# rsinghlab/GNN-Tumor-Seg

Measured on AMD Instinct MI355X. Metric: supervoxel-graphs/sec training, 7xSAGE-pool-256, 15k-node graphs, higher is better.
Workload: dtype f32

## Files before the change

gnn-tumor-seg_amd/csrc/gts_rows.h:

```cpp
#pragma once
#include <type_traits>

#include "gts_common.h"

namespace gts {

constexpr int kUnroll = 8;

__device__ __forceinline__ float mad(float w, float v, float acc) { return __builtin_fmaf(w, v, acc); }

typedef float v2f __attribute__((ext_vector_type(2)));
constexpr float kEluSplit = -0.35f, kLog2e = 1.44269504088896340736f;
constexpr float kEluC2 = 0.5f, kEluC3 = 1.0f / 6.0f, kEluC4 = 1.0f / 24.0f, kEluC5 = 1.0f / 120.0f, kEluC6 = 1.0f / 720.0f,
                kEluC7 = 1.0f / 5040.0f;
__device__ __forceinline__ float elu_expm1(float x) {
  float q = __builtin_fmaf(kEluC7, x, kEluC6);
  q = __builtin_fmaf(q, x, kEluC5);
  q = __builtin_fmaf(q, x, kEluC4);
  q = __builtin_fmaf(q, x, kEluC3);
  q = __builtin_fmaf(q, x, kEluC2);
  const float small = __builtin_fmaf(x * x, q, x);
  const float large = __builtin_amdgcn_exp2f(x * kLog2e) - 1.0f;
  return x < kEluSplit ? large : small;
}
__device__ __forceinline__ v2f elu_expm1_pair(v2f x) {
  v2f q = __builtin_elementwise_fma(v2f{kEluC7, kEluC7}, x, v2f{kEluC6, kEluC6});
  q = __builtin_elementwise_fma(q, x, v2f{kEluC5, kEluC5});
  q = __builtin_elementwise_fma(q, x, v2f{kEluC4, kEluC4});
  q = __builtin_elementwise_fma(q, x, v2f{kEluC3, kEluC3});
  q = __builtin_elementwise_fma(q, x, v2f{kEluC2, kEluC2});
  const v2f small = __builtin_elementwise_fma(x * x, q, x);
  const v2f arg = x * v2f{kLog2e, kLog2e};
  const v2f large = v2f{__builtin_amdgcn_exp2f(arg.x), __builtin_amdgcn_exp2f(arg.y)} - v2f{1.0f, 1.0f};
  return v2f{x.x < kEluSplit ? large.x : small.x, x.y < kEluSplit ? large.y : small.y};
}

template <int LPR>
__device__ __forceinline__ int owned_row(int s, int seq, int n_rows) {
  constexpr int kRowsPerWave = kWave / LPR;
  const int lane = threadIdx.x & (kWave - 1);
  const int wave = threadIdx.x / kWave;
  const int tile = xcd_contiguous_tile(blockIdx.x, gridDim.x);
  int v = ((tile * kWavesPerBlock + wave) * seq + s) * kRowsPerWave + lane / LPR;
  if constexpr (LPR == kWave) v = __builtin_amdgcn_readfirstlane(v);
  return v < n_rows ? v : -1;
}

template <int VEC, int LPR, typename Body>
__device__ __forceinline__ void for_columns(int n_feat, Body&& body) {
  const int gl = (threadIdx.x & (kWave - 1)) % LPR;
  for (int c0 = 0; c0 < n_feat; c0 += LPR * VEC) {
    const int c = c0 + gl * VEC;
    const bool active = c < n_feat;
    body(active ? c : 0, active);
  }
}

template <int N>
using IC = std::integral_constant<int, N>;

template <int LPR, typename Body>
__device__ __forceinline__ void for_chunks(int beg, int end, Body&& body) {
  if constexpr (LPR == kWave) {
    int k = beg;
    for (; k + kUnroll <= end; k += kUnroll) body(IC<kUnroll>{}, k);
    switch (end - k) {
      case 1: body(IC<1>{}, k); break;
      case 2: body(IC<2>{}, k); break;
      case 3: body(IC<3>{}, k); break;
      case 4: body(IC<4>{}, k); break;
      case 5: body(IC<5>{}, k); break;
      case 6: body(IC<6>{}, k); break;
      case 7: body(IC<7>{}, k); break;
      default: break;
    }
  } else {
    for (int k = beg; k < end; k += kUnroll) body(IC<kUnroll>{}, k);
  }
}

template <int LPR, int CNT>
struct Chunk {
  int reg;
  const int32_t* __restrict__ p;
  int k, last;
  __device__ __forceinline__ Chunk(const int32_t* __restrict__ arr, int k_, int end) : p(arr), k(k_), last(end - 1) {
    if constexpr (LPR == kWave) {
      const int lane = threadIdx.x & (kWave - 1);
      reg = lane < CNT ? arr[k_ + lane] : 0;
    } else {
      reg = 0;
    }
  }
  __device__ __forceinline__ int operator[](int j) const {
    if constexpr (LPR == kWave) {
      return __builtin_amdgcn_readlane(reg, j);
    } else {
      return p[min(k + j, last)];
    }
  }
  __device__ __forceinline__ bool valid(int j) const {
    if constexpr (LPR == kWave) return true;
    return k + j <= last;
  }
};

inline int g_spmm_seq = 0;
inline int g_project_nt = 1;
inline int g_spmm_nt = -1;
inline int g_cluster_nt = -1;
inline int g_gat_walk = 1;
inline int g_cluster_ring = 0;
inline int g_cluster_per_cu = 0;
inline int g_gat_cluster_waves = 0;
inline int g_cluster_dealing = 0;
inline int g_gat_cluster_dealing = 0;
inline int g_gat_cluster_group = 0;
inline int g_cluster_consumers = 0;

inline int pick_seq(int64_t n_rows, int rows_per_wave_step, int preferred) {
  if (g_spmm_seq > 0) return g_spmm_seq;
  if (preferred > 0) return preferred;
  const int64_t steps = (n_rows + rows_per_wave_step - 1) / rows_per_wave_step;
  int seq = 1;
  while (seq < 4 && steps / (seq * 2) >= 8192) seq *= 2;
  return seq;
}

struct Geometry {
  int vec, lpr, seq;
  dim3 grid;
};

inline Geometry make_geometry(int64_t n_rows, int64_t n_feat, int preferred_seq = 0) {
  Geometry g;
  g.vec = (n_feat % 4 == 0) ? 4 : 1;
  g.lpr = lanes_per_row(n_feat / g.vec);
  const int rows_per_step = kWave / g.lpr;
  g.seq = pick_seq(n_rows, rows_per_step, preferred_seq);
  const int64_t rows_per_block = static_cast<int64_t>(rows_per_step) * g.seq * kWavesPerBlock;
  g.grid = dim3(static_cast<unsigned>((n_rows + rows_per_block - 1) / rows_per_block));
  return g;
}

inline bool bad_shape(int64_t n_rows, int64_t n_feat) {
  return n_rows < 0 || n_feat <= 0 || n_rows >= (1LL << 31) || n_feat >= (1LL << 24);
}

}

#define GTS_DISPATCH_LPR(VEC_, LPR_VAL, ...)                \
  switch (LPR_VAL) {                                        \
    case 1: { constexpr int LPR = 1; __VA_ARGS__; } break;  \
    case 2: { constexpr int LPR = 2; __VA_ARGS__; } break;  \
    case 4: { constexpr int LPR = 4; __VA_ARGS__; } break;  \
    case 8: { constexpr int LPR = 8; __VA_ARGS__; } break;  \
    case 16: { constexpr int LPR = 16; __VA_ARGS__; } break; \
    case 32: { constexpr int LPR = 32; __VA_ARGS__; } break; \
    default: { constexpr int LPR = 64; __VA_ARGS__; } break; \
  }

#define GTS_DISPATCH_GEOM(G, ...)                                   \
  if ((G).vec == 4) {                                               \
    constexpr int VEC = 4;                                          \
    GTS_DISPATCH_LPR(4, (G).lpr, __VA_ARGS__)                       \
  } else {                                                          \
    constexpr int VEC = 1;                                          \
    GTS_DISPATCH_LPR(1, (G).lpr, __VA_ARGS__)                       \
  }
```

gnn-tumor-seg_amd/csrc/gts_spmm.hip:

```cpp
#include "gts_rows.h"

namespace gts {
namespace {

template <int ARGB>
struct ArgTraits;
template <>
struct ArgTraits<1> {
  using T = uint8_t;
  static constexpr int kNone = 0xFF;
};
template <>
struct ArgTraits<4> {
  using T = int32_t;
  static constexpr int kNone = -1;
};

template <int VEC, int ARGB>
__device__ __forceinline__ void store_slots(void* arg, size_t off, const int (&slot)[VEC]) {
  if constexpr (ARGB == 1) {
    uint8_t* p = static_cast<uint8_t*>(arg) + off;
    if constexpr (VEC == 4) {
      const uint32_t w = (slot[0] & 0xFF) | ((slot[1] & 0xFF) << 8) | ((slot[2] & 0xFF) << 16) |
                         (static_cast<uint32_t>(slot[3] & 0xFF) << 24);
      *reinterpret_cast<uint32_t*>(p) = w;
    } else {
      p[0] = static_cast<uint8_t>(slot[0]);
    }
  } else if constexpr (ARGB == 4) {
    int32_t* p = static_cast<int32_t*>(arg) + off;
    if constexpr (VEC == 4) {
      *reinterpret_cast<int4*>(p) = make_int4(slot[0], slot[1], slot[2], slot[3]);
    } else {
      p[0] = slot[0];
    }
  }
}

template <int VEC, int ARGB>
__device__ __forceinline__ void load_slots(const void* arg, size_t off, int (&slot)[VEC]) {
  if constexpr (ARGB == 1) {
    const uint8_t* p = static_cast<const uint8_t*>(arg) + off;
    if constexpr (VEC == 4) {
      const uint32_t w = *reinterpret_cast<const uint32_t*>(p);
      slot[0] = w & 0xFF;
      slot[1] = (w >> 8) & 0xFF;
      slot[2] = (w >> 16) & 0xFF;
      slot[3] = w >> 24;
    } else {
      slot[0] = p[0];
    }
  } else {
    const int32_t* p = static_cast<const int32_t*>(arg) + off;
    if constexpr (VEC == 4) {
      const int4 w = *reinterpret_cast<const int4*>(p);
      slot[0] = w.x, slot[1] = w.y, slot[2] = w.z, slot[3] = w.w;
    } else {
      slot[0] = p[0];
    }
  }
}

template <int VEC, int LPR, int ARGB>
__global__ __launch_bounds__(kBlock) void spmm_max_fwd_kernel(
    const int32_t* __restrict__ indptr, const int32_t* __restrict__ indices,
    const float* __restrict__ x, float* __restrict__ out, void* __restrict__ arg, int n_dst,
    int n_feat, int seq, int nt, int relu_input) {
  for (int s = 0; s < seq; ++s) {
    const int v = owned_row<LPR>(s, seq, n_dst);
    if (v < 0) continue;
    const int beg = indptr[v], end = indptr[v + 1];
    for_columns<VEC, LPR>(n_feat, [&](int c, bool active) {
      float best[VEC];
      int slot[VEC];
#pragma unroll
      for (int t = 0; t < VEC; ++t) best[t] = -INFINITY, slot[t] = -1;
      for_chunks<LPR>(beg, end, [&](auto cnt_c, int k) {
        constexpr int CNT = decltype(cnt_c)::value;
        const Chunk<LPR, CNT> src(indices, k, end);
        Vec<VEC> val[CNT];
#pragma unroll
        for (int j = 0; j < CNT; ++j)
          val[j] = Vec<VEC>::load(x + static_cast<size_t>(src[j]) * n_feat + c);
#pragma unroll
        for (int j = 0; j < CNT; ++j) {
          if (src.valid(j)) {
#pragma unroll
            for (int t = 0; t < VEC; ++t) {
              if (best[t] < val[j].v[t]) best[t] = val[j].v[t], slot[t] = k + j - beg;
            }
          }
        }
      });
      Vec<VEC> o;
#pragma unroll
      for (int t = 0; t < VEC; ++t) {
        const bool dead = isinf(best[t]);
        o.v[t] = dead ? 0.0f : best[t];
        slot[t] = (dead || (relu_input && !(best[t] > 0.0f))) ? -1 : slot[t];
      }
      const size_t off = static_cast<size_t>(v) * n_feat + c;
      if (active) {
        if (nt & 1) o.store_nt(out + off); else o.store(out + off);
        if constexpr (ARGB != 0) store_slots<VEC, ARGB>(arg, off, slot);
      }
    });
  }
}

template <int VEC, int LPR, int ARGB>
__global__ __launch_bounds__(kBlock) void spmm_max_bwd_kernel(
    const int32_t* __restrict__ t_indptr, const int32_t* __restrict__ t_indices,
    const int32_t* __restrict__ t_slot, const float* __restrict__ gout,
    const void* __restrict__ arg, const float* __restrict__ relu_src, float* __restrict__ gx,
    int n_src, int n_feat, int seq, int nt) {
  for (int s = 0; s < seq; ++s) {
    const int u = owned_row<LPR>(s, seq, n_src);
    if (u < 0) continue;
    const int beg = t_indptr[u], end = t_indptr[u + 1];
    for_columns<VEC, LPR>(n_feat, [&](int c, bool active) {
      float acc[VEC];
#pragma unroll
      for (int t = 0; t < VEC; ++t) acc[t] = 0.0f;
      for_chunks<LPR>(beg, end, [&](auto cnt_c, int k) {
        constexpr int CNT = decltype(cnt_c)::value;
        const Chunk<LPR, CNT> dst(t_indices, k, end);
        const Chunk<LPR, CNT> slt(t_slot, k, end);
        Vec<VEC> g[CNT];
        int win[CNT][VEC];
        int want[CNT];
#pragma unroll
        for (int j = 0; j < CNT; ++j) {
          const size_t off = static_cast<size_t>(dst[j]) * n_feat + c;
          want[j] = slt[j];
          g[j] = Vec<VEC>::load(gout + off);
          load_slots<VEC, ARGB>(arg, off, win[j]);
        }
#pragma unroll
        for (int j = 0; j < CNT; ++j) {
          if (dst.valid(j)) {
#pragma unroll
            for (int t = 0; t < VEC; ++t) acc[t] += (win[j][t] == want[j]) ? g[j].v[t] : 0.0f;
          }
        }
      });
      const size_t off = static_cast<size_t>(u) * n_feat + c;
      Vec<VEC> o;
      if (relu_src != nullptr) {
        const Vec<VEC> p = (nt & 2) ? Vec<VEC>::load_nt(relu_src + off) : Vec<VEC>::load(relu_src + off);
#pragma unroll
        for (int t = 0; t < VEC; ++t) o.v[t] = p.v[t] > 0.0f ? acc[t] : 0.0f;
      } else {
#pragma unroll
        for (int t = 0; t < VEC; ++t) o.v[t] = acc[t];
      }
      if (active) { if (nt & 1) o.store_nt(gx + off); else o.store(gx + off); }
    });
  }
}

template <int VEC, int LPR, bool DIV_IN>
__global__ __launch_bounds__(kBlock) void spmm_sum_kernel(
    const int32_t* __restrict__ indptr, const int32_t* __restrict__ indices,
    const float* __restrict__ x, float* __restrict__ out, const float* __restrict__ div_in,
    const float* __restrict__ div_out, const float* __restrict__ accum, int add_self, int n_out, int n_feat,
    int seq) {
  for (int s = 0; s < seq; ++s) {
    const int v = owned_row<LPR>(s, seq, n_out);
    if (v < 0) continue;
    const int beg = indptr[v], end = indptr[v + 1];
    for_columns<VEC, LPR>(n_feat, [&](int c, bool active) {
      float acc[VEC];
#pragma unroll
      for (int t = 0; t < VEC; ++t) acc[t] = 0.0f;
      for_chunks<LPR>(beg, end, [&](auto cnt_c, int k) {
        constexpr int CNT = decltype(cnt_c)::value;
        const Chunk<LPR, CNT> src(indices, k, end);
        Vec<VEC> val[CNT];
        float d[CNT];
#pragma unroll
        for (int j = 0; j < CNT; ++j) {
          const int u = src[j];
          d[j] = DIV_IN ? div_in[u] : 1.0f;
          val[j] = Vec<VEC>::load(x + static_cast<size_t>(u) * n_feat + c);
        }
#pragma unroll
        for (int j = 0; j < CNT; ++j) {
          if (src.valid(j)) {
#pragma unroll
            for (int t = 0; t < VEC; ++t) acc[t] += DIV_IN ? val[j].v[t] / d[j] : val[j].v[t];
          }
        }
      });
      const size_t off = static_cast<size_t>(v) * n_feat + c;
      if (add_self) {
        const Vec<VEC> self = Vec<VEC>::load(x + off);
        const float d = DIV_IN ? div_in[v] : 1.0f;
#pragma unroll
        for (int t = 0; t < VEC; ++t) acc[t] += DIV_IN ? self.v[t] / d : self.v[t];
      }
      Vec<VEC> o;
      const float dv = div_out != nullptr ? div_out[v] : 1.0f;
#pragma unroll
      for (int t = 0; t < VEC; ++t) o.v[t] = div_out != nullptr ? acc[t] / dv : acc[t];
      if (accum != nullptr) {
        const Vec<VEC> other = Vec<VEC>::load(accum + off);
#pragma unroll
        for (int t = 0; t < VEC; ++t) o.v[t] = other.v[t] + o.v[t];
      }
      if (active) o.store(out + off);
    });
  }
}

}
}

extern "C" int32_t gts_spmm_max_fwd_f32(const int32_t* indptr, const int32_t* indices,
                                        const float* x, float* out, void* arg,
                                        int32_t arg_bytes, int32_t relu_input, int64_t n_dst,
                                        int64_t n_feat, void* stream) {
  using namespace gts;
  if (!indptr || !x || !out || (arg_bytes != 0 && !arg)) return GTS_ERR_NULL;
  if (bad_shape(n_dst, n_feat)) return GTS_ERR_SHAPE;
  if (arg_bytes != 0 && arg_bytes != 1 && arg_bytes != 4) return GTS_ERR_ARGKIND;
  if (n_dst == 0) return GTS_OK;
  const Geometry g = make_geometry(n_dst, n_feat, 2);
  const int nt = g_spmm_nt < 0 ? 1 : g_spmm_nt;
  hipStream_t st = static_cast<hipStream_t>(stream);
  const int nd = static_cast<int>(n_dst), nf = static_cast<int>(n_feat);
  GTS_DISPATCH_GEOM(g, {
    if (arg_bytes == 0)
      spmm_max_fwd_kernel<VEC, LPR, 0><<<g.grid, kBlock, 0, st>>>(indptr, indices, x, out, arg, nd, nf, g.seq, nt, relu_input);
    else if (arg_bytes == 1)
      spmm_max_fwd_kernel<VEC, LPR, 1><<<g.grid, kBlock, 0, st>>>(indptr, indices, x, out, arg, nd, nf, g.seq, nt, relu_input);
    else
      spmm_max_fwd_kernel<VEC, LPR, 4><<<g.grid, kBlock, 0, st>>>(indptr, indices, x, out, arg, nd, nf, g.seq, nt, relu_input);
  })
  return launch_status();
}

extern "C" int32_t gts_spmm_max_bwd_f32(const int32_t* t_indptr, const int32_t* t_indices,
                                        const int32_t* t_slot, const float* gout,
                                        const void* arg, int32_t arg_bytes,
                                        const float* relu_src, float* gx, int64_t n_src,
                                        int64_t n_feat, void* stream) {
  using namespace gts;
  if (!t_indptr || !gout || !arg || !gx) return GTS_ERR_NULL;
  if (bad_shape(n_src, n_feat)) return GTS_ERR_SHAPE;
  if (arg_bytes != 1 && arg_bytes != 4) return GTS_ERR_ARGKIND;
  if (n_src == 0) return GTS_OK;
  const Geometry g = make_geometry(n_src, n_feat, 1);
  const int nt = g_spmm_nt < 0 ? 0 : g_spmm_nt;
  hipStream_t st = static_cast<hipStream_t>(stream);
  const int ns = static_cast<int>(n_src), nf = static_cast<int>(n_feat);
  GTS_DISPATCH_GEOM(g, {
    if (arg_bytes == 1)
      spmm_max_bwd_kernel<VEC, LPR, 1><<<g.grid, kBlock, 0, st>>>(t_indptr, t_indices, t_slot, gout, arg, relu_src, gx, ns, nf, g.seq, nt);
    else
      spmm_max_bwd_kernel<VEC, LPR, 4><<<g.grid, kBlock, 0, st>>>(t_indptr, t_indices, t_slot, gout, arg, relu_src, gx, ns, nf, g.seq, nt);
  })
  return launch_status();
}

extern "C" int32_t gts_spmm_sum_f32(const int32_t* indptr, const int32_t* indices,
                                    const float* x, float* out, const float* div_in,
                                    const float* div_out, const float* accum, int32_t add_self,
                                    int64_t n_out, int64_t n_feat, void* stream) {
  using namespace gts;
  if (!indptr || !x || !out) return GTS_ERR_NULL;
  if (bad_shape(n_out, n_feat)) return GTS_ERR_SHAPE;
  if (n_out == 0) return GTS_OK;
  const Geometry g = make_geometry(n_out, n_feat);
  hipStream_t st = static_cast<hipStream_t>(stream);
  const int no = static_cast<int>(n_out), nf = static_cast<int>(n_feat);
  GTS_DISPATCH_GEOM(g, {
    if (div_in != nullptr)
      spmm_sum_kernel<VEC, LPR, true><<<g.grid, kBlock, 0, st>>>(indptr, indices, x, out, div_in, div_out, accum, add_self, no, nf, g.seq);
    else
      spmm_sum_kernel<VEC, LPR, false><<<g.grid, kBlock, 0, st>>>(indptr, indices, x, out, div_in, div_out, accum, add_self, no, nf, g.seq);
  })
  return launch_status();
}
```

gnn-tumor-seg_amd/csrc/gts_spmm_cluster.hip:

```cpp
#include <algorithm>
#include <queue>
#include <vector>

#include "gts_cluster.h"

namespace gts {
namespace {

struct ClusterArgs {
  const int32_t* rec;
  RecLayout layout;
  int n_clusters, max_srcs;
  const float* table;
  const uint8_t* winners;
  float* out;
  uint8_t* arg;
  unsigned table_bytes, winners_bytes;
  int relu_input, nt;
  int ring, slot_bytes, image_off, win_off;
  int deal_off;
  unsigned* counters;
};

template <int ARGB, int WHATIF = 0>
__device__ __forceinline__ int reduce_max_rows(const ClusterArgs& a, const int32_t* l_rec, const unsigned char* image,
                                               int part, int first, int step) {
  const int lane = threadIdx.x & (kWave - 1), half = lane >> 5, hl = lane & 31;
  const int n_rows = l_rec[0];
  const uint32_t* info = reinterpret_cast<const uint32_t*>(l_rec + a.layout.eoff);
  const uint2* loc = reinterpret_cast<const uint2*>(l_rec + a.layout.loc);
  const unsigned char* mine = image + hl * 16;
  int trips = 0;
  for (int j0 = 2 * first; j0 < n_rows; j0 += 2 * step, ++trips) {
    const int j = j0 + half;
    const bool have = j < n_rows;
    const uint32_t ri = have ? info[j] : 0u;
    const int c0 = ri & 0xFFFF, deg = ri >> 16;
    const int deg_w = max(__builtin_amdgcn_readlane(deg, 0), __builtin_amdgcn_readlane(deg, 32));
    float best[4];
    int slot[4];
#pragma unroll
    for (int t = 0; t < 4; ++t) best[t] = -INFINITY, slot[t] = -1;
    for (int c = 0; 8 * c < deg_w && WHATIF != 4; ++c) {
      const bool mine_too = 8 * c < deg;
      const uint2 w = loc[mine_too ? c0 + c : c0];
      for_count(min(8, deg_w - 8 * c), [&](auto cnt_c) {
        constexpr int CNT = decltype(cnt_c)::value;
        constexpr int FIRST = CNT > 6 ? 6 : CNT;
        float4 val[FIRST];
#pragma unroll
        for (int q = 0; q < FIRST; ++q) val[q] = *reinterpret_cast<const float4*>(mine + chunk_byte(w, q) * kHalfBytes);
#pragma unroll
        for (int q = 0; q < FIRST; ++q) {
          const float v4[4] = {val[q].x, val[q].y, val[q].z, val[q].w};
#pragma unroll
          for (int t = 0; t < 4; ++t) {
            const bool up = mine_too && best[t] < v4[t];
            best[t] = up ? v4[t] : best[t];
            slot[t] = up ? 8 * c + q : slot[t];
          }
        }
        if constexpr (CNT > FIRST) {
          float4 rest[CNT - FIRST];
#pragma unroll
          for (int q = FIRST; q < CNT; ++q) rest[q - FIRST] = *reinterpret_cast<const float4*>(mine + chunk_byte(w, q) * kHalfBytes);
#pragma unroll
          for (int q = FIRST; q < CNT; ++q) {
            const float v4[4] = {rest[q - FIRST].x, rest[q - FIRST].y, rest[q - FIRST].z, rest[q - FIRST].w};
#pragma unroll
            for (int t = 0; t < 4; ++t) {
              const bool up = mine_too && best[t] < v4[t];
              best[t] = up ? v4[t] : best[t];
              slot[t] = up ? 8 * c + q : slot[t];
            }
          }
        }
      });
    }
    Vec<4> o;
#pragma unroll
    for (int t = 0; t < 4; ++t) {
      const bool dead = isinf(best[t]);
      o.v[t] = dead ? 0.0f : best[t];
      slot[t] = (dead || (a.relu_input && !(best[t] > 0.0f))) ? -1 : slot[t];
    }
    if (WHATIF == 3) {
      if (o.v[0] == 123.456f) a.out[0] = static_cast<float>(slot[0] + slot[1] + slot[2] + slot[3]) + o.v[1] + o.v[2] + o.v[3];
    } else if (have) {
      const size_t off = static_cast<size_t>(l_rec[a.layout.rows + j]) * kF + part * (kF / 2) + hl * 4;
      if (a.nt & 1) o.store_nt(a.out + off); else o.store(a.out + off);
      if constexpr (ARGB == 1) {
        const uint32_t w = (slot[0] & 0xFF) | ((slot[1] & 0xFF) << 8) | ((slot[2] & 0xFF) << 16) |
                           (static_cast<uint32_t>(slot[3] & 0xFF) << 24);
        *reinterpret_cast<uint32_t*>(a.arg + off) = w;
      }
    }
  }
  return trips * (ARGB == 1 ? 2 : 1);
}

__device__ __forceinline__ int reduce_winner_rows(const ClusterArgs& a, const int32_t* l_rec, const unsigned char* image,
                                                  const unsigned char* winners, int part, int first, int step) {
  const int lane = threadIdx.x & (kWave - 1), half = lane >> 5, hl = lane & 31;
  const int n_rows = l_rec[0];
  const uint32_t* info = reinterpret_cast<const uint32_t*>(l_rec + a.layout.eoff);
  const uint2* loc = reinterpret_cast<const uint2*>(l_rec + a.layout.loc);
  const uint2* tag = reinterpret_cast<const uint2*>(l_rec + a.layout.tag);
  const unsigned char* my_g = image + hl * 16;
  const unsigned char* my_w = winners + hl * 4;
  int trips = 0;
  for (int j0 = 2 * first; j0 < n_rows; j0 += 2 * step, ++trips) {
    const int j = j0 + half;
    const bool have = j < n_rows;
    const uint32_t ri = have ? info[j] : 0u;
    const int c0 = ri & 0xFFFF, deg = ri >> 16;
    const int deg_a = __builtin_amdgcn_readlane(deg, 0), deg_b = __builtin_amdgcn_readlane(deg, 32);
    const int deg_w = max(deg_a, deg_b);
    float acc[4] = {0.f, 0.f, 0.f, 0.f};
    if (deg_a == deg_b && deg_w <= 8) {
      if (deg_w > 0) {
        const uint2 w = loc[c0], tg = tag[c0];
        for_count(deg_w, [&](auto cnt_c) {
          constexpr int CNT = decltype(cnt_c)::value;
          constexpr int FIRST = CNT > 6 ? 6 : CNT;
          auto group = [&](auto q0_c, auto n_c) {
            constexpr int Q0 = decltype(q0_c)::value, N = decltype(n_c)::value;
            float4 g[N];
            uint32_t win[N];
#pragma unroll
            for (int q = 0; q < N; ++q) {
              const unsigned s = chunk_byte(w, Q0 + q);
              g[q] = *reinterpret_cast<const float4*>(my_g + s * kHalfBytes);
              win[q] = *reinterpret_cast<const uint32_t*>(my_w + s * kArgHalfBytes);
            }
#pragma unroll
            for (int q = 0; q < N; ++q) {
              const unsigned want = chunk_byte(tg, Q0 + q);
              acc[0] += (win[q] & 0xFF) == want ? g[q].x : 0.0f;
              acc[1] += ((win[q] >> 8) & 0xFF) == want ? g[q].y : 0.0f;
              acc[2] += ((win[q] >> 16) & 0xFF) == want ? g[q].z : 0.0f;
              acc[3] += (win[q] >> 24) == want ? g[q].w : 0.0f;
            }
          };
          group(IC<0>{}, IC<FIRST>{});
          if constexpr (CNT > FIRST) group(IC<FIRST>{}, IC<CNT - FIRST>{});
        });
      }
    } else {
      for (int c = 0; 8 * c < deg_w; ++c) {
        const int at = 8 * c < deg ? c0 + c : c0;
        const uint2 w = loc[at], tg = tag[at];
        for_count(min(8, deg_w - 8 * c), [&](auto cnt_c) {
          constexpr int CNT = decltype(cnt_c)::value;
          constexpr int FIRST = CNT > 6 ? 6 : CNT;
          auto group = [&](auto q0_c, auto n_c) {
            constexpr int Q0 = decltype(q0_c)::value, N = decltype(n_c)::value;
            float4 g[N];
            uint32_t win[N];
#pragma unroll
            for (int q = 0; q < N; ++q) {
              const unsigned s = chunk_byte(w, Q0 + q);
              g[q] = *reinterpret_cast<const float4*>(my_g + s * kHalfBytes);
              win[q] = *reinterpret_cast<const uint32_t*>(my_w + s * kArgHalfBytes);
            }
#pragma unroll
            for (int q = 0; q < N; ++q) {
              const unsigned want = chunk_byte(tg, Q0 + q);
              const bool live = 8 * c + Q0 + q < deg;
              const float g4[4] = {g[q].x, g[q].y, g[q].z, g[q].w};
#pragma unroll
              for (int t = 0; t < 4; ++t) acc[t] += (live && ((win[q] >> (8 * t)) & 0xFF) == want) ? g4[t] : 0.0f;
            }
          };
          group(IC<0>{}, IC<FIRST>{});
          if constexpr (CNT > FIRST) group(IC<FIRST>{}, IC<CNT - FIRST>{});
        });
      }
    }
    if (have) {
      const size_t off = static_cast<size_t>(l_rec[a.layout.rows + j]) * kF + part * (kF / 2) + hl * 4;
      const Vec<4> o{{acc[0], acc[1], acc[2], acc[3]}};
      if (a.nt & 1) o.store_nt(a.out + off); else o.store(a.out + off);
    }
  }
  return trips;
}

template <typename Dma, typename SrcOf>
__device__ __forceinline__ void gather_winner_halves(const Dma& dma, int part, unsigned char* image,
                                                     int n_srcs, int first, int step, SrcOf&& src_of) {
  const int l8 = threadIdx.x & 7;
  for (int i = first; i < n_srcs; i += step) {
    const unsigned voff = static_cast<unsigned>(src_of(i)) * static_cast<unsigned>(kF) +
                          static_cast<unsigned>(part) * kArgHalfBytes + l8 * 16u;
    dma(image + i * kArgHalfBytes, voff);
  }
}

template <bool BWD, int ARGB, int WHATIF = 0, int DEPTH = 1, bool DEAL = false>
__global__ __launch_bounds__(1024, BWD ? 6 : 8) void spmm_cluster_stream_kernel(const ClusterArgs a) {
  extern __shared__ __attribute__((aligned(16))) unsigned char lds[];
  const int lane = threadIdx.x & (kWave - 1);
  const int wave = __builtin_amdgcn_readfirstlane(threadIdx.x / kWave);
  const int n_waves = blockDim.x / kWave;
  const int xcd = blockIdx.x & 7, j = blockIdx.x >> 3, per_xcd = gridDim.x >> 3;
  const long long n_units = 2LL * a.n_clusters;
  const int lo = static_cast<int>(n_units * xcd / 8), hi = static_cast<int>(n_units * (xcd + 1) / 8);
  constexpr bool dynamic = DEAL;
  const int n_static = lo + j < hi ? (hi - lo - j + per_xcd - 1) / per_xcd : 0;
  if (!dynamic && n_static == 0) return;
  const int clo = static_cast<int>(static_cast<long long>(a.n_clusters) * xcd / 8);
  const int span = static_cast<int>(static_cast<long long>(a.n_clusters) * (xcd + 1) / 8) - clo;
  const int words = a.layout.words;
  const int pieces = (words + 255) / 256;
  const int rec_bytes = 1024 * pieces, image_bytes = a.slot_bytes - a.image_off;
  constexpr int depth = DEPTH, n_images = DEPTH + 1, n_recs = DEPTH + 2;
  unsigned char* images = lds + n_recs * rec_bytes;
  const RawDma rr(a.rec, static_cast<unsigned>(a.n_clusters) * words * 4u);
  const RawDma rt(a.table, a.table_bytes);
  const RawDma rw(a.winners, BWD ? a.winners_bytes : 0);
  constexpr int PIPE = DEPTH + 2;
  int u_unit[dynamic ? PIPE : 1];
#pragma unroll
  for (int q = 0; q < (dynamic ? PIPE : 1); ++q) u_unit[q] = -1;
  int32_t* l_deal = reinterpret_cast<int32_t*>(lds + a.deal_off);
  auto next_unit = [&](int deal_slot) {
    if constexpr (dynamic) {
#pragma unroll
      for (int q = PIPE - 1; q > 0; --q) u_unit[q] = u_unit[q - 1];
      const unsigned idx = static_cast<unsigned>(__builtin_amdgcn_readfirstlane(l_deal[deal_slot]));
      const unsigned part = idx >= static_cast<unsigned>(span) ? 1u : 0u;
      u_unit[0] = idx < 2u * static_cast<unsigned>(span) ? static_cast<int>(((clo + idx - part * span) << 1) | part) : -1;
    }
  };
  auto unit_at = [&](int k, int newest) {
    if constexpr (dynamic) {
      return u_unit[k];
    } else {
      const int t = newest - k;
      return t < n_static ? lo + j + t * per_xcd : -1;
    }
  };
  auto take = [&](int count) {
    unsigned base = 0;
    if (lane == 0) base = __hip_atomic_fetch_add(a.counters + 32 * xcd, static_cast<unsigned>(count), __ATOMIC_RELAXED, __HIP_MEMORY_SCOPE_AGENT);
    return base;
  };
  auto publish = [&](unsigned taken, int count, int slot0) {
    if (lane == 0) {
      for (int q = 0; q < count; ++q) l_deal[slot0 + q] = static_cast<int>(taken + q);
    }
  };
  auto fetch_record = [&](int t, int unit) {
    if (wave < pieces) {
      const unsigned cluster = static_cast<unsigned>(unit) >> 1;
      const int word = 256 * wave + 4 * lane;
      const unsigned voff = word < words ? (cluster * static_cast<unsigned>(words) + word) * 4u : 0xFFFFFFF0u;
      rr(lds + (t % n_recs) * rec_bytes + 1024 * wave, voff);
    }
  };
  auto issue_gathers = [&](int t, int unit) {
    const int32_t* l_rec = reinterpret_cast<const int32_t*>(lds + (t % n_recs) * rec_bytes);
    unsigned char* image = images + (t % n_images) * image_bytes;
    const int n_srcs = l_rec[1];
    const int part = unit & 1;
    const int half = lane >> 5;
    const int last = pad4(a.max_srcs) - 1;
    const int32_t ids = l_rec[a.layout.srcs + min(2 * (wave + n_waves * (lane >> 1)) + (lane & 1), last)];
    int k = 0;
    gather_halves(rt, part, image, n_srcs, 2 * wave, 2 * n_waves, [&](int) {
      const int s0 = __builtin_amdgcn_readlane(ids, 2 * k), s1 = __builtin_amdgcn_readlane(ids, 2 * k + 1);
      ++k;
      return half ? s1 : s0;
    });
    if constexpr (BWD) {
      const int32_t ids8 = l_rec[a.layout.srcs + min(8 * (wave + n_waves * (lane >> 3)) + (lane & 7), last)];
      int k8 = 0;
      gather_winner_halves(rw, part, image + ((a.max_srcs + 1) & ~1) * kHalfBytes, n_srcs, 8 * wave, 8 * n_waves, [&](int) {
        const int32_t id = __builtin_amdgcn_ds_bpermute(4 * (8 * k8 + (lane >> 3)), ids8);
        ++k8;
        return id;
      });
      return k + k8;
    }
    return k;
  };

  if constexpr (dynamic) {
    if (wave == n_waves - 1) {
      const unsigned first = take(PIPE);
      publish(first, PIPE - 1, 0);
      publish(first + (PIPE - 1), 1, 6);
    }
    barrier_all();
  }
  unsigned taken = 0;
#pragma unroll
  for (int t = 0; t <= depth; ++t) {
    next_unit(t);
    if (unit_at(0, t) >= 0) fetch_record(t, unit_at(0, t));
  }
  barrier_all();
  int pending_gathers = 0, stores = 0;
#pragma unroll
  for (int t = 0; t < depth; ++t) pending_gathers = (WHATIF != 1 && unit_at(depth - t, depth) >= 0) ? issue_gathers(t, unit_at(depth - t, depth)) : 0;
  if (depth == 1) pending_gathers = 0;
  unsigned long long phase[4] = {0, 0, 0, 0}, stamp = 0;
  auto lap = [&](int which) {
    if constexpr (WHATIF == 9) {
      const unsigned long long now = __builtin_amdgcn_s_memtime();
      phase[which] += now - stamp;
      stamp = now;
    }
  };
  if constexpr (WHATIF == 9) stamp = __builtin_amdgcn_s_memtime();
  int it = 0;
  for (; dynamic || it < n_static; ++it) {
    wait_vm_all_but(pending_gathers + stores);
    if constexpr (dynamic) {
      if (it > 0 && wave == n_waves - 1) publish(taken, 1, 6 + (it & 1));
    }
    lap(0);
    barrier_lds();
    lap(1);
    next_unit(6 + (it & 1));
    const int newest = it + depth + 1;
    const int unit_now = unit_at(PIPE - 1, newest);
    if constexpr (dynamic) {
      if (unit_now < 0) break;
    }
    if constexpr (dynamic) {
      if (wave == n_waves - 1) taken = take(1);
    }
    if constexpr (DEPTH == 1) {
      if (unit_at(1, newest) >= 0 && WHATIF != 1) issue_gathers(it + 1, unit_at(1, newest));
      if (unit_at(0, newest) >= 0) fetch_record(it + 2, unit_at(0, newest));
    } else {
      if (unit_at(0, newest) >= 0) fetch_record(it + depth + 1, unit_at(0, newest));
      pending_gathers = (unit_at(1, newest) >= 0 && WHATIF != 1) ? issue_gathers(it + depth, unit_at(1, newest)) : 0;
    }
    lap(2);
    const int32_t* l_rec = reinterpret_cast<const int32_t*>(lds + (it % n_recs) * rec_bytes);
    const unsigned char* image = images + (it % n_images) * image_bytes;
    const int part = unit_now & 1;
    if constexpr (WHATIF == 2)
      stores = 0;
    else if constexpr (WHATIF >= 3 && WHATIF <= 4 && !BWD)
      stores = WHATIF == 3 ? (reduce_max_rows<ARGB, WHATIF>(a, l_rec, image, part, wave, n_waves), 0)
                           : reduce_max_rows<ARGB, WHATIF>(a, l_rec, image, part, wave, n_waves);
    else if constexpr (BWD)
      stores = reduce_winner_rows(a, l_rec, image, image + ((a.max_srcs + 1) & ~1) * kHalfBytes, part, wave, n_waves);
    else
      stores = reduce_max_rows<ARGB>(a, l_rec, image, part, wave, n_waves);
    lap(3);
  }
  if constexpr (WHATIF == 9) {
    if (threadIdx.x == 0) {
      unsigned long long* dbg = reinterpret_cast<unsigned long long*>(a.arg) + 8 * static_cast<size_t>(blockIdx.x);
      for (int q = 0; q < 4; ++q) dbg[q] = phase[q];
      dbg[4] = static_cast<unsigned long long>(it);
    }
  }
  if (dynamic && threadIdx.x == 0) {
    unsigned* done = a.counters + 32 * xcd + 16;
    if (__hip_atomic_fetch_add(done, 1u, __ATOMIC_RELAXED, __HIP_MEMORY_SCOPE_AGENT) == static_cast<unsigned>(per_xcd) - 1u) {
      __hip_atomic_store(a.counters + 32 * xcd, 0u, __ATOMIC_RELAXED, __HIP_MEMORY_SCOPE_AGENT);
      __hip_atomic_store(done, 0u, __ATOMIC_RELAXED, __HIP_MEMORY_SCOPE_AGENT);
    }
  }
}

struct LdsPlan {
  int slot_bytes, image_off, win_off;
};
inline LdsPlan lds_plan(int max_rows, int max_srcs, int loc_words, bool bwd) {
  const RecLayout l = rec_layout(max_rows, max_srcs, loc_words, bwd);
  LdsPlan p;
  p.image_off = (l.words * 4 + 15) & ~15;
  const int image = ((max_srcs + 1) & ~1) * kHalfBytes;
  p.win_off = p.image_off + image;
  p.slot_bytes = p.win_off + (bwd ? ((max_srcs + 7) & ~7) * kArgHalfBytes : 0);
  return p;
}

struct ClusterGeometry {
  int64_t wg_lds, grid;
  int depth, waves;
  bool deals;
};
inline ClusterGeometry cluster_geometry(int64_t n_clusters, int words, int slot_bytes, int image_off, bool bwd, bool whatif) {
  ClusterGeometry g;
  const int64_t units = 2LL * n_clusters;
  const int64_t rec_slot = 1024LL * ((words + 255) / 256), image = slot_bytes - image_off;
  g.depth = (g_cluster_ring == 2 && !whatif && 4 * rec_slot + 3 * image + 64 <= kMaxLds) ? 2 : 1;
  g.wg_lds = (g.depth + 2) * rec_slot + (g.depth + 1) * image + 64;
  g.waves = g_cluster_consumers > 0 ? std::min(16, g_cluster_consumers) : (bwd ? 12 : 16);
  const int auto_per_cu = (bwd && units <= 24LL * device_cus()) ? 3 : 2;
  const int per_cu = static_cast<int>(std::max<int64_t>(1, std::min<int64_t>(g_cluster_per_cu > 0 ? g_cluster_per_cu : auto_per_cu, kMaxLds / std::max<int64_t>(1, g.wg_lds))));
  g.grid = static_cast<int64_t>(device_cus()) * per_cu;
  g.grid = std::max<int64_t>(8, std::min(g.grid, (units + 7) / 8 * 8)) / 8 * 8;
  g.deals = g_cluster_dealing == 1 || (g_cluster_dealing == 0 && units >= 16 * g.grid);
  return g;
}

template <bool BWD, int ARGB, int WHATIF = 0>
inline int launch_cluster(ClusterArgs a, int max_rows, int loc_words, hipStream_t st) {
  const LdsPlan p = lds_plan(max_rows, a.max_srcs, loc_words, BWD);
  a.image_off = p.image_off, a.win_off = p.win_off, a.slot_bytes = p.slot_bytes;
  if (p.slot_bytes > kMaxLds) return GTS_ERR_SHAPE;
  const int64_t units = 2LL * a.n_clusters;
  {
    const ClusterGeometry geo = cluster_geometry(a.n_clusters, a.layout.words, p.slot_bytes, p.image_off, BWD, WHATIF != 0);
    const int depth = geo.depth, waves = geo.waves;
    const int64_t wg_lds = geo.wg_lds, grid = geo.grid;
    a.deal_off = static_cast<int>(wg_lds) - 64;
    if (wg_lds > kMaxLds || a.layout.words > 512) return GTS_ERR_SHAPE;
    a.ring = depth;
    if (a.max_srcs > 64 * waves) return GTS_ERR_SHAPE;
    if (!geo.deals) a.counters = nullptr;
    static const bool once = (allow_big_lds(spmm_cluster_stream_kernel<BWD, ARGB, WHATIF, 1, false>),
                              allow_big_lds(spmm_cluster_stream_kernel<BWD, ARGB, WHATIF, 1, true>),
                              allow_big_lds(spmm_cluster_stream_kernel<BWD, ARGB, WHATIF == 0 ? 0 : WHATIF, WHATIF == 0 ? 2 : 1, false>),
                              allow_big_lds(spmm_cluster_stream_kernel<BWD, ARGB, WHATIF == 0 ? 0 : WHATIF, WHATIF == 0 ? 2 : 1, true>), true);
    (void)once;
    const dim3 g3(static_cast<unsigned>(grid));
    if constexpr (WHATIF == 0) {
      if (depth == 2) {
        if (a.counters != nullptr) spmm_cluster_stream_kernel<BWD, ARGB, 0, 2, true><<<g3, waves * kWave, wg_lds, st>>>(a);
        else spmm_cluster_stream_kernel<BWD, ARGB, 0, 2, false><<<g3, waves * kWave, wg_lds, st>>>(a);
        return launch_status();
      }
    }
    if (a.counters != nullptr) spmm_cluster_stream_kernel<BWD, ARGB, WHATIF, 1, true><<<g3, waves * kWave, wg_lds, st>>>(a);
    else spmm_cluster_stream_kernel<BWD, ARGB, WHATIF, 1, false><<<g3, waves * kWave, wg_lds, st>>>(a);
    return launch_status();
  }
}

}
}

extern "C" int64_t gts_cluster_record_words(int32_t max_rows, int32_t max_srcs, int32_t loc_words, int32_t with_tag) {
  if (max_rows < 1 || max_srcs < 1 || loc_words < 0 || loc_words % 4 != 0) return -1;
  return gts::rec_layout(max_rows, max_srcs, loc_words, with_tag != 0).words;
}

extern "C" int32_t gts_cluster_schedule(const int32_t* indptr, const int32_t* indices, const int32_t* t_indptr,
                                        const int32_t* t_indices, const int32_t* edge_tag, int64_t n_rows,
                                        int32_t max_rows, int32_t max_srcs, int32_t max_edges, int32_t* rec,
                                        int64_t rec_capacity, int64_t* n_clusters, int64_t* n_staged,
                                        int32_t* max_cluster_edges) {
  using namespace gts;
  if (!indptr || !t_indptr || !n_clusters || !n_staged || !max_cluster_edges) return GTS_ERR_NULL;
  if (n_rows < 0 || n_rows >= (1LL << 31)) return GTS_ERR_SHAPE;
  if (max_rows < 1 || max_srcs < 1 || max_srcs > 256 || max_edges < 1 || max_edges > 65535) return GTS_ERR_ARGKIND;
  const int n = static_cast<int>(n_rows);
  if (n > 0 && (!indices || !t_indices) && indptr[n] > 0) return GTS_ERR_NULL;
  if (n > 0) {
    if (indptr[0] != 0 || t_indptr[0] != 0) return GTS_ERR_SHAPE;
    for (int v = 0; v < n; ++v)
      if (indptr[v + 1] < indptr[v] || t_indptr[v + 1] < t_indptr[v]) return GTS_ERR_SHAPE;
    if (indptr[n] != t_indptr[n]) return GTS_ERR_SHAPE;
    const int e_all = indptr[n];
    for (int k = 0; k < e_all; ++k)
      if (indices[k] < 0 || indices[k] >= n || t_indices[k] < 0 || t_indices[k] >= n) return GTS_ERR_SHAPE;
  }
  for (int v = 0; v < n; ++v) {
    const int deg = indptr[v + 1] - indptr[v];
    if (deg > max_srcs || ((deg + 7) & ~7) > max_edges || deg > 65535) return GTS_ERR_SHAPE;
  }
  if (edge_tag != nullptr) {
    const int e = n > 0 ? indptr[n] : 0;
    for (int k = 0; k < e; ++k)
      if (edge_tag[k] < 0 || edge_tag[k] > 255) return GTS_ERR_SHAPE;
  }
  const int loc_words = pad4((max_edges + 3) / 4);
  const RecLayout L = rec_layout(max_rows, max_srcs, loc_words, edge_tag != nullptr);
  if (L.words > 64 * kRecRegs) return GTS_ERR_ARGKIND;
  std::vector<uint8_t> assigned(n, 0);
  std::vector<int> gain(n, 0), stamp(n, -1);
  std::vector<int> local(n, -1), lstamp(n, -1);
  using Cand = std::pair<int, int>;
  std::priority_queue<Cand> heap;
  std::priority_queue<int, std::vector<int>, std::greater<int>> seeds;
  std::vector<int> rows, srcs, touched;
  int next_unassigned = 0, most_edges = 0;
  int64_t n_cl = 0, staged = 0;
  while (true) {
    int seed = -1;
    while (!seeds.empty()) {
      const int s = seeds.top();
      seeds.pop();
      if (!assigned[s]) { seed = s; break; }
    }
    if (seed < 0) {
      while (next_unassigned < n && assigned[next_unassigned]) ++next_unassigned;
      if (next_unassigned == n) break;
      seed = next_unassigned;
    }
    const int cl = static_cast<int>(n_cl);
    rows.clear(), srcs.clear(), touched.clear();
    int n_e = 0;
    while (!heap.empty()) heap.pop();
    heap.push({0, -seed});
    stamp[seed] = cl, gain[seed] = 0;
    bool full = false, misfit = false;
    while (!full) {
      if (heap.empty()) {
        if (misfit) break;
        while (next_unassigned < n && assigned[next_unassigned]) ++next_unassigned;
        if (next_unassigned == n) break;
        const int s = next_unassigned;
        if (stamp[s] != cl) stamp[s] = cl, gain[s] = 0;
        heap.push({gain[s], -s});
      }
      const Cand top = heap.top();
      heap.pop();
      const int v = -top.second;
      if (assigned[v] || stamp[v] != cl || gain[v] != top.first) continue;
      const int beg = indptr[v], end = indptr[v + 1];
      int fresh = 0;
      for (int k = beg; k < end; ++k) {
        const int u = indices[k];
        if (lstamp[u] != cl) lstamp[u] = cl, local[u] = -1;
        if (local[u] == -1) local[u] = -2, ++fresh;
      }
      const int padded = (end - beg + 7) & ~7;
      const bool fits = static_cast<int>(rows.size()) < max_rows &&
                        static_cast<int>(srcs.size()) + fresh <= max_srcs && n_e + padded <= max_edges;
      if (!fits) {
        for (int k = beg; k < end; ++k)
          if (local[indices[k]] == -2) local[indices[k]] = -1;
        if (rows.empty()) return GTS_ERR_SHAPE;
        misfit = true;
        continue;
      }
      assigned[v] = 1;
      rows.push_back(v);
      n_e += padded;
      for (int k = beg; k < end; ++k) {
        const int u = indices[k];
        if (local[u] != -2) continue;
        local[u] = static_cast<int>(srcs.size());
        srcs.push_back(u);
        for (int q = t_indptr[u]; q < t_indptr[u + 1]; ++q) {
          const int w = t_indices[q];
          if (assigned[w]) continue;
          if (stamp[w] != cl) stamp[w] = cl, gain[w] = 0, touched.push_back(w);
          ++gain[w];
          heap.push({gain[w], -w});
        }
      }
      if (static_cast<int>(rows.size()) >= max_rows) full = true;
    }
    for (int w : touched)
      if (!assigned[w]) seeds.push(w);
    most_edges = std::max(most_edges, n_e);
    staged += static_cast<int64_t>(srcs.size());
    if (rec != nullptr && n_cl < rec_capacity) {
      std::sort(rows.begin(), rows.end());
      int32_t* r = rec + n_cl * L.words;
      std::fill(r, r + L.words, 0);
      r[0] = static_cast<int32_t>(rows.size()), r[1] = static_cast<int32_t>(srcs.size()), r[2] = n_e;
      uint8_t* loc = reinterpret_cast<uint8_t*>(r + L.loc);
      uint8_t* tag = reinterpret_cast<uint8_t*>(r + L.tag);
      int e_at = 0;
      for (size_t i = 0; i < rows.size(); ++i) {
        const int v = rows[i], deg = indptr[v + 1] - indptr[v];
        r[L.rows + i] = v;
        r[L.eoff + i] = static_cast<int32_t>(static_cast<uint32_t>(e_at / 8) | (static_cast<uint32_t>(deg) << 16));
        for (int k = indptr[v]; k < indptr[v + 1]; ++k, ++e_at) {
          loc[e_at] = static_cast<uint8_t>(local[indices[k]]);
          if (edge_tag != nullptr) tag[e_at] = static_cast<uint8_t>(edge_tag[k]);
        }
        for (; e_at % 8 != 0; ++e_at) {
          loc[e_at] = loc[e_at - 1];
          if (edge_tag != nullptr) tag[e_at] = tag[e_at - 1];
        }
      }
      for (int i = 0; i < pad4(max_srcs); ++i)
        r[L.srcs + i] = srcs.empty() ? 0 : srcs[std::min<size_t>(i, srcs.size() - 1)];
    }
    ++n_cl;
  }
  *n_clusters = n_cl;
  *n_staged = staged;
  *max_cluster_edges = most_edges;
  return GTS_OK;
}

extern "C" int64_t gts_cluster_lds_bytes(int32_t max_rows, int32_t max_srcs, int32_t loc_words, int32_t kind) {
  if (max_rows < 1 || max_srcs < 1 || loc_words < 0 || loc_words % 4 != 0 || (kind != 0 && kind != 1)) return -1;
  return gts::lds_plan(max_rows, max_srcs, loc_words, kind == 1).slot_bytes;
}

namespace {
inline bool bad_cluster_shape(int64_t n_clusters, int32_t max_rows, int32_t max_srcs, int32_t loc_words, bool tag,
                              int64_t n_rows, int64_t n_feat) {
  if (n_feat != gts::kF || n_rows < 0 || n_rows * gts::kF * 4 >= (1LL << 32) || n_clusters < 0 || n_clusters >= (1 << 30))
    return true;
  if (max_rows < 1 || max_srcs < 1 || max_srcs > 256 || loc_words < 0 || loc_words % 4 != 0 || loc_words > 16384) return true;
  return gts::rec_layout(max_rows, max_srcs, loc_words, tag).words > 64 * gts::kRecRegs;
}
}

extern "C" int32_t gts_cluster_uses_counters(int64_t n_clusters, int32_t max_rows, int32_t max_srcs, int32_t loc_words, int32_t backward) {
  using namespace gts;
  if (n_clusters <= 0 || max_rows < 1 || max_srcs < 1 || loc_words < 0) return 0;
  const LdsPlan p = lds_plan(max_rows, max_srcs, loc_words, backward != 0);
  return cluster_geometry(n_clusters, rec_layout(max_rows, max_srcs, loc_words, backward != 0).words, p.slot_bytes, p.image_off, backward != 0, false).deals ? 1 : 0;
}

extern "C" int32_t gts_spmm_max_fwd_cluster_f32(const int32_t* rec, int64_t n_clusters, int32_t max_rows, int32_t max_srcs,
                                                int32_t loc_words, const float* x, float* out, void* arg,
                                                int32_t arg_bytes, int32_t relu_input, int64_t n_rows, int64_t n_feat,
                                                uint32_t* counters, void* stream) {
  using namespace gts;
  if (!rec || !x || !out || (arg_bytes != 0 && !arg)) return GTS_ERR_NULL;
  if (bad_cluster_shape(n_clusters, max_rows, max_srcs, loc_words, false, n_rows, n_feat)) return GTS_ERR_SHAPE;
  if (arg_bytes != 0 && arg_bytes != 1) return GTS_ERR_ARGKIND;
  if (n_clusters == 0) return GTS_OK;
  ClusterArgs a{};
  a.rec = rec, a.layout = rec_layout(max_rows, max_srcs, loc_words, false);
  a.n_clusters = static_cast<int>(n_clusters), a.max_srcs = max_srcs;
  a.table = x, a.out = out, a.arg = static_cast<uint8_t*>(arg), a.counters = counters;
  a.table_bytes = static_cast<unsigned>(n_rows * kF * 4);
  a.relu_input = relu_input, a.nt = g_cluster_nt < 0 ? 1 : g_cluster_nt;
  hipStream_t st = static_cast<hipStream_t>(stream);
  return arg_bytes == 0 ? launch_cluster<false, 0>(a, max_rows, loc_words, st) : launch_cluster<false, 1>(a, max_rows, loc_words, st);
}

extern "C" int32_t gts_spmm_max_bwd_cluster_f32(const int32_t* rec, int64_t n_clusters, int32_t max_rows, int32_t max_srcs,
                                                int32_t loc_words, const float* gout, const void* arg, int32_t arg_bytes,
                                                float* gx, int64_t n_rows, int64_t n_feat, uint32_t* counters, void* stream) {
  using namespace gts;
  if (!rec || !gout || !arg || !gx) return GTS_ERR_NULL;
  if (bad_cluster_shape(n_clusters, max_rows, max_srcs, loc_words, true, n_rows, n_feat)) return GTS_ERR_SHAPE;
  if (arg_bytes != 1) return GTS_ERR_ARGKIND;
  if (n_clusters == 0) return GTS_OK;
  ClusterArgs a{};
  a.rec = rec, a.layout = rec_layout(max_rows, max_srcs, loc_words, true);
  a.n_clusters = static_cast<int>(n_clusters), a.max_srcs = max_srcs;
  a.table = gout, a.winners = static_cast<const uint8_t*>(arg), a.out = gx, a.counters = counters;
  a.table_bytes = static_cast<unsigned>(n_rows * kF * 4), a.winners_bytes = static_cast<unsigned>(n_rows * kF);
  a.nt = g_cluster_nt < 0 ? 1 : g_cluster_nt;
  return launch_cluster<true, 1>(a, max_rows, loc_words, static_cast<hipStream_t>(stream));
}
```

gnn-tumor-seg_amd/csrc/gts_stack.hip:

```cpp
#include <algorithm>
#include <vector>

#include "gts_common.h"

namespace {

constexpr int kMaxLayers = 64;
constexpr int kMaxWgradProblems = 32;
constexpr int kFlagChain = 1, kFlagReluBits = 2, kFlagTransposedIgrad = 4;

inline int64_t align256(int64_t bytes) { return (bytes + 255) & ~255LL; }

inline bool bad_stack(int64_t n_rows, const int64_t* widths, int32_t n_layers) {
  if (!widths || n_layers < 1 || n_layers > kMaxLayers || n_rows < 0 || n_rows >= (1LL << 31)) return true;
  for (int i = 0; i <= n_layers; ++i)
    if (widths[i] <= 0 || widths[i] % 4 != 0 || widths[i] >= (1 << 20)) return true;
  return false;
}

struct FwdPlan {
  int64_t m[kMaxLayers], arg[kMaxLayers], out[kMaxLayers], bits[kMaxLayers];
  int64_t p[2];
  int64_t wp[kMaxLayers][3];
  int64_t counters;
  int64_t total;
};

inline bool packs(int64_t out_cols) { return out_cols > 128; }

inline FwdPlan plan_forward(int64_t n, const int64_t* w, int n_layers, bool training, int arg_bytes, int flags) {
  FwdPlan p{};
  int64_t at = 0, widest = 0;
  auto take = [&](int64_t bytes) { const int64_t o = at; at += align256(bytes); return o; };
  for (int i = 0; i < n_layers; ++i) {
    const bool last = i == n_layers - 1;
    widest = std::max(widest, w[i]);
    p.m[i] = take(4 * n * w[i]);
    p.arg[i] = training ? take(static_cast<int64_t>(arg_bytes) * n * w[i]) : -1;
    p.out[i] = take(4 * n * w[i + 1]);
    const bool bits = (flags & kFlagReluBits) && training && !last && gts_relu_bits_pay(n, w[i + 1]) == 1;
    p.bits[i] = bits ? take(gts_relu_bits_bytes(n, w[i + 1])) : -1;
  }
  p.p[0] = take(4 * n * widest);
  p.p[1] = take(4 * n * widest);
  for (int i = 0; i < n_layers; ++i) {
    p.wp[i][0] = packs(w[i]) ? take(4 * gts_packed_weight_floats(w[i], w[i])) : -1;
    p.wp[i][1] = packs(w[i + 1]) ? take(4 * gts_packed_weight_floats(w[i + 1], w[i])) : -1;
    p.wp[i][2] = packs(w[i + 1]) ? take(4 * gts_packed_weight_floats(w[i + 1], w[i])) : -1;
  }
  p.counters = take(4 * GTS_CLUSTER_COUNTER_WORDS);
  p.total = at;
  return p;
}

inline bool chainable(int64_t n, int64_t k0, int64_t k1, int64_t n2) {
  return n % 4 == 0 && k0 % 4 == 0 && k1 % 4 == 0 && n <= 256 && n2 <= 256;
}

struct Schedule {
  const int32_t* rec;
  int64_t clusters;
  int32_t rows, srcs, loc_words;
};

inline bool turns(int64_t rows, int64_t cols) { return cols >= 128 && rows % 4 == 0 && cols % 4 == 0; }

struct BwdPlan {
  int64_t wt[kMaxLayers][3];
  int64_t wtp[kMaxLayers][3];
  int64_t g[kMaxLayers], gp[kMaxLayers];
  int64_t gm[2];
  int64_t workspace, workspace_bytes;
  int64_t counters;
  int64_t total;
};

struct WgradGroup {
  int64_t n, k;
  std::vector<const float*> g, a;
  std::vector<float*> gw, gb;
};

inline BwdPlan plan_backward(int64_t n, const int64_t* w, int n_layers, int flags) {
  BwdPlan p{};
  int64_t at = 0, widest = 0;
  auto take = [&](int64_t bytes) { const int64_t o = at; at += align256(bytes); return o; };
  const bool t = (flags & kFlagTransposedIgrad) != 0;
  for (int i = 0; i < n_layers; ++i) {
    const int64_t fin = w[i], fout = w[i + 1];
    widest = std::max(widest, fin);
    p.wt[i][0] = t && turns(fin, fin) ? take(4 * fin * fin) : -1;
    p.wt[i][1] = t && turns(fout, fin) ? take(4 * fout * fin) : -1;
    p.wt[i][2] = t && turns(fout, fin) ? take(4 * fout * fin) : -1;
    p.wtp[i][0] = p.wt[i][0] >= 0 ? take(4 * gts_packed_weight_floats(fin, fin)) : -1;
    p.wtp[i][1] = p.wt[i][1] >= 0 ? take(4 * gts_packed_weight_floats(fin, fout)) : -1;
    p.wtp[i][2] = p.wt[i][2] >= 0 ? take(4 * gts_packed_weight_floats(fin, fout)) : -1;
    p.g[i] = i > 0 ? take(4 * n * fin) : -1;
    p.gp[i] = take(4 * n * fin);
  }
  p.gm[0] = take(4 * n * widest);
  p.gm[1] = take(4 * n * widest);
  struct Key { int64_t n, k; int count; };
  std::vector<Key> groups;
  auto add = [&](int64_t nn, int64_t kk) {
    for (auto& gk : groups)
      if (gk.n == nn && gk.k == kk) { ++gk.count; return; }
    groups.push_back({nn, kk, 1});
  };
  for (int i = n_layers - 1; i >= 0; --i) add(w[i], w[i]), add(w[i + 1], w[i]), add(w[i + 1], w[i]);
  int64_t ws = 0;
  if (n > 0)
    for (const auto& gk : groups)
      for (int first = 0; first < gk.count; first += kMaxWgradProblems)
        ws = std::max(ws, gts_linear_bwd_weight_workspace(n, gk.n, gk.k, std::min(kMaxWgradProblems, gk.count - first)));
  p.workspace_bytes = ws;
  p.workspace = take(ws);
  p.counters = take(4 * GTS_CLUSTER_COUNTER_WORDS);
  p.total = at;
  return p;
}

#define GTS_TRY(call)                    \
  do {                                   \
    const int32_t code_ = (call);        \
    if (code_ != GTS_OK) return code_;   \
  } while (0)

}

extern "C" int64_t gts_sage_pool_stack_fwd_arena(int64_t n_rows, const int64_t* widths, int32_t n_layers, int32_t training,
                                                 int32_t arg_bytes, int32_t flags, int64_t* offsets) {
  if (bad_stack(n_rows, widths, n_layers) || (training && arg_bytes != 1 && arg_bytes != 4)) return -1;
  const FwdPlan p = plan_forward(n_rows, widths, n_layers, training != 0, arg_bytes, flags);
  if (offsets != nullptr) {
    for (int i = 0; i < n_layers; ++i)
      offsets[4 * i] = p.m[i], offsets[4 * i + 1] = p.arg[i], offsets[4 * i + 2] = p.out[i], offsets[4 * i + 3] = p.bits[i];
    offsets[4 * n_layers] = p.p[0], offsets[4 * n_layers + 1] = p.p[1];
  }
  return p.total;
}

extern "C" int32_t gts_sage_pool_stack_fwd_f32(const int32_t* indptr, const int32_t* indices, const int32_t* sched_rec,
                                               int64_t sched_clusters, int32_t sched_rows, int32_t sched_srcs,
                                               int32_t sched_loc_words, const float* x, const float* const* params,
                                               int64_t n_rows, const int64_t* widths, int32_t n_layers, int32_t training,
                                               int32_t arg_bytes, int32_t flags, void* arena, int64_t arena_bytes,
                                               void* stream) {
  if (!indptr || !x || !params || !arena) return GTS_ERR_NULL;
  if (bad_stack(n_rows, widths, n_layers)) return GTS_ERR_SHAPE;
  if (training && arg_bytes != 1 && arg_bytes != 4) return GTS_ERR_ARGKIND;
  for (int i = 0; i < 5 * n_layers; ++i)
    if (!params[i]) return GTS_ERR_NULL;
  const bool train = training != 0;
  const FwdPlan plan = plan_forward(n_rows, widths, n_layers, train, arg_bytes, flags);
  if (arena_bytes < plan.total) return GTS_ERR_SHAPE;
  if (n_rows == 0) return GTS_OK;
  char* base = static_cast<char*>(arena);
  auto f32 = [&](int64_t off) { return reinterpret_cast<float*>(base + off); };
  uint32_t* counters = nullptr;
  if (sched_rec != nullptr && gts_cluster_uses_counters(sched_clusters, sched_rows, sched_srcs, sched_loc_words, 0) != 0) {
    counters = reinterpret_cast<uint32_t*>(base + plan.counters);
    if (hipMemsetAsync(counters, 0, 4 * GTS_CLUSTER_COUNTER_WORDS, static_cast<hipStream_t>(stream)) != hipSuccess) return GTS_ERR_SHAPE;
  }
  {
    struct Batch { int64_t rows, cols; std::vector<const float*> src; std::vector<float*> dst; };
    std::vector<Batch> batches;
    for (int i = 0; i < n_layers; ++i) {
      const int64_t fin = widths[i], fout = widths[i + 1];
      const int64_t shape[3][2] = {{fin, fin}, {fout, fin}, {fout, fin}};
      const int which[3] = {0, 2, 3};
      for (int q = 0; q < 3; ++q) {
        if (plan.wp[i][q] < 0) continue;
        Batch* b = nullptr;
        for (auto& c : batches)
          if (c.rows == shape[q][0] && c.cols == shape[q][1]) b = &c;
        if (b == nullptr) batches.push_back({shape[q][0], shape[q][1], {}, {}}), b = &batches.back();
        b->src.push_back(params[5 * i + which[q]]);
        b->dst.push_back(f32(plan.wp[i][q]));
      }
    }
    for (const auto& b : batches)
      GTS_TRY(gts_pack_weights_f32(b.src.data(), b.dst.data(), nullptr, static_cast<int32_t>(b.src.size()), b.rows, b.cols, 0,
                                   stream));
  }
  auto wp = [&](int i, int q) -> const float* { return plan.wp[i][q] >= 0 ? f32(plan.wp[i][q]) : nullptr; };
  const float* h = x;
  float* p = nullptr;
  int cur = 0;
  for (int i = 0; i < n_layers; ++i) {
    const float* w_pool = params[5 * i];
    const float* b_pool = params[5 * i + 1];
    const float* w_self = params[5 * i + 2];
    const float* w_neigh = params[5 * i + 3];
    const float* bias = params[5 * i + 4];
    const int64_t fin = widths[i], fout = widths[i + 1];
    const bool last = i == n_layers - 1;
    if (p == nullptr) {
      p = f32(plan.p[cur]);
      const float* packed[2] = {wp(i, 0), nullptr};
      GTS_TRY(gts_linear_fwd_f32(h, w_pool, nullptr, nullptr, b_pool, p, n_rows, fin, fin, 0, 1, nullptr, packed, stream));
    }
    float* m = f32(plan.m[i]);
    void* arg = train ? static_cast<void*>(base + plan.arg[i]) : nullptr;
    const int ab = train ? arg_bytes : 0;
    if (sched_rec != nullptr && fin == 256 && ab != 4 && n_rows * 1024 < (1LL << 32)) {
      GTS_TRY(gts_spmm_max_fwd_cluster_f32(sched_rec, sched_clusters, sched_rows, sched_srcs, sched_loc_words, p, m, arg, ab,
                                           1, n_rows, fin, counters, stream));
    } else {
      GTS_TRY(gts_spmm_max_fwd_f32(indptr, indices, p, m, arg, ab, 1, n_rows, fin, stream));
    }
    uint64_t* bits = plan.bits[i] >= 0 ? reinterpret_cast<uint64_t*>(base + plan.bits[i]) : nullptr;
    float* out = f32(plan.out[i]);
    if ((flags & kFlagChain) && !last && chainable(fout, fin, fin, fout)) {
      float* p_next = f32(plan.p[cur ^ 1]);
      const float* packed[3] = {wp(i, 1), wp(i, 2), wp(i + 1, 0)};
      GTS_TRY(gts_linear_fwd_chain_f32(h, w_self, m, w_neigh, bias, out, params[5 * (i + 1)], params[5 * (i + 1) + 1], p_next,
                                       n_rows, fout, fin, fin, 1, fout, 1, bits, packed, stream));
      p = p_next, cur ^= 1;
    } else {
      const float* packed[2] = {wp(i, 1), wp(i, 2)};
      GTS_TRY(gts_linear_fwd_f32(h, w_self, m, w_neigh, bias, out, n_rows, fout, fin, fin, last ? 0 : 1, bits, packed, stream));
      p = nullptr;
    }
    h = out;
  }
  return GTS_OK;
}

extern "C" int64_t gts_sage_pool_stack_bwd_scratch(int64_t n_rows, const int64_t* widths, int32_t n_layers, int32_t flags) {
  if (bad_stack(n_rows, widths, n_layers)) return -1;
  return plan_backward(n_rows, widths, n_layers, flags).total;
}

extern "C" int32_t gts_sage_pool_stack_bwd_f32(const int32_t* t_indptr, const int32_t* t_indices, const int32_t* t_slot,
                                               const int32_t* sched_rec, int64_t sched_clusters, int32_t sched_rows,
                                               int32_t sched_srcs, int32_t sched_loc_words, const float* gout, const float* x,
                                               const float* const* params, int64_t n_rows, const int64_t* widths,
                                               int32_t n_layers, int32_t arg_bytes, int32_t flags, const void* fwd_arena,
                                               float* const* grads, float* gx, void* scratch, int64_t scratch_bytes,
                                               void* stream) {
  if (!t_indptr || !gout || !x || !params || !fwd_arena || !grads || !scratch) return GTS_ERR_NULL;
  if (bad_stack(n_rows, widths, n_layers)) return GTS_ERR_SHAPE;
  if (arg_bytes != 1 && arg_bytes != 4) return GTS_ERR_ARGKIND;
  for (int i = 0; i < 5 * n_layers; ++i)
    if (!params[i] || !grads[i]) return GTS_ERR_NULL;
  hipStream_t st = static_cast<hipStream_t>(stream);
  if (n_rows == 0) {
    for (int i = 0; i < n_layers; ++i) {
      const int64_t fin = widths[i], fout = widths[i + 1];
      const int64_t sizes[5] = {fin * fin, fin, fout * fin, fout * fin, fout};
      for (int q = 0; q < 5; ++q)
        if (hipMemsetAsync(grads[5 * i + q], 0, 4 * sizes[q], st) != hipSuccess) return gts::launch_status();
    }
    return GTS_OK;
  }
  const FwdPlan fwd = plan_forward(n_rows, widths, n_layers, true, arg_bytes, flags);
  const BwdPlan plan = plan_backward(n_rows, widths, n_layers, flags);
  if (scratch_bytes < plan.total) return GTS_ERR_SHAPE;
  const char* acts = static_cast<const char*>(fwd_arena);
  char* base = static_cast<char*>(scratch);
  auto f32 = [&](int64_t off) { return reinterpret_cast<float*>(base + off); };
  uint32_t* counters = nullptr;
  if (sched_rec != nullptr && gts_cluster_uses_counters(sched_clusters, sched_rows, sched_srcs, sched_loc_words, 1) != 0) {
    counters = reinterpret_cast<uint32_t*>(base + plan.counters);
    if (hipMemsetAsync(counters, 0, 4 * GTS_CLUSTER_COUNTER_WORDS, static_cast<hipStream_t>(stream)) != hipSuccess) return GTS_ERR_SHAPE;
  }
  auto act = [&](int64_t off) { return reinterpret_cast<const float*>(acts + off); };
  auto input_of = [&](int i) { return i == 0 ? x : act(fwd.out[i - 1]); };

  {
    struct Batch { int64_t rows, cols; std::vector<const float*> src; std::vector<float*> dst, packed; };
    std::vector<Batch> batches;
    for (int i = 0; i < n_layers; ++i) {
      const int64_t fin = widths[i], fout = widths[i + 1];
      const int64_t shape[3][2] = {{fin, fin}, {fout, fin}, {fout, fin}};
      const int which[3] = {0, 2, 3};
      for (int q = 0; q < 3; ++q) {
        if (plan.wt[i][q] < 0) continue;
        Batch* b = nullptr;
        for (auto& c : batches)
          if (c.rows == shape[q][0] && c.cols == shape[q][1]) b = &c;
        if (b == nullptr) batches.push_back({shape[q][0], shape[q][1], {}, {}, {}}), b = &batches.back();
        b->src.push_back(params[5 * i + which[q]]);
        b->dst.push_back(f32(plan.wt[i][q]));
        b->packed.push_back(f32(plan.wtp[i][q]));
      }
    }
    for (const auto& b : batches)
      GTS_TRY(gts_pack_weights_f32(b.src.data(), b.packed.data(), b.dst.data(), static_cast<int32_t>(b.src.size()), b.rows,
                                   b.cols, 1, stream));
  }
  auto wt = [&](int i, int q) -> const float* { return plan.wt[i][q] >= 0 ? f32(plan.wt[i][q]) : nullptr; };
  auto wtp = [&](int i, int q) -> const float* { return plan.wtp[i][q] >= 0 ? f32(plan.wtp[i][q]) : nullptr; };

  auto igrad = [&](const float* g0, const float* w0, const float* w0t, int64_t n0, const float* g1, const float* w1,
                   const float* w1t, int64_t n1, const float* relu_mask, const uint64_t* relu_bits, float* gin,
                   int64_t k, const float* w0tp, const float* w1tp) -> int32_t {
    if (w0t != nullptr && (g1 == nullptr || w1t != nullptr)) {
      const float* packed[2] = {w0tp, g1 ? w1tp : nullptr};
      return gts_linear_bwd_input_t_f32(g0, w0t, g1, g1 ? w1t : nullptr, relu_mask, relu_mask ? relu_bits : nullptr, gin,
                                        n_rows, k, n0, g1 ? n1 : 0, packed, stream);
    }
    return gts_linear_bwd_input_f32(g0, w0, g1, g1 ? w1 : nullptr, relu_mask, gin, n_rows, k, n0, g1 ? n1 : 0, stream);
  };

  std::vector<WgradGroup> groups;
  auto defer = [&](const float* g, int64_t n, const float* a, int64_t k, float* gw, float* gb) {
    WgradGroup* grp = nullptr;
    for (auto& c : groups)
      if (c.n == n && c.k == k) grp = &c;
    if (grp == nullptr) groups.push_back({n, k, {}, {}, {}, {}}), grp = &groups.back();
    grp->g.push_back(g), grp->a.push_back(a), grp->gw.push_back(gw), grp->gb.push_back(gb);
  };

  const float* g = gout;
  const float* gm = nullptr;
  int cur = 0;
  for (int i = n_layers - 1; i >= 0; --i) {
    const float* w_pool = params[5 * i];
    const float* w_self = params[5 * i + 2];
    const float* w_neigh = params[5 * i + 3];
    const int64_t fin = widths[i], fout = widths[i + 1];
    const float* h = input_of(i);
    const float* m = act(fwd.m[i]);
    const void* arg = acts + fwd.arg[i];
    if (gm == nullptr) {
      float* buf = f32(plan.gm[cur]);
      GTS_TRY(igrad(g, w_neigh, wt(i, 2), fout, nullptr, nullptr, nullptr, 0, nullptr, nullptr, buf, fin, wtp(i, 2), nullptr));
      gm = buf;
    }
    float* gp = f32(plan.gp[i]);
    if (sched_rec != nullptr && fin == 256 && arg_bytes == 1 && n_rows * 1024 < (1LL << 32)) {
      GTS_TRY(gts_spmm_max_bwd_cluster_f32(sched_rec, sched_clusters, sched_rows, sched_srcs, sched_loc_words, gm, arg, 1, gp,
                                           n_rows, fin, counters, stream));
    } else {
      GTS_TRY(gts_spmm_max_bwd_f32(t_indptr, t_indices, t_slot, gm, arg, arg_bytes, nullptr, gp, n_rows, fin, stream));
    }
    gm = nullptr;
    defer(gp, fin, h, fin, grads[5 * i], grads[5 * i + 1]);
    defer(g, fout, h, fin, grads[5 * i + 2], grads[5 * i + 4]);
    defer(g, fout, m, fin, grads[5 * i + 3], nullptr);
    if (i > 0) {
      const int64_t below_in = widths[i - 1];
      const uint64_t* hbits = fwd.bits[i - 1] >= 0 ? reinterpret_cast<const uint64_t*>(acts + fwd.bits[i - 1]) : nullptr;
      float* g_next = f32(plan.g[i]);
      const float* below_t = wt(i - 1, 2);
      if ((flags & kFlagChain) && wt(i, 1) && wt(i, 0) && below_t && chainable(fin, fout, fin, below_in)) {
        float* gm_next = f32(plan.gm[cur ^ 1]);
        const float* packed[3] = {wtp(i, 1), wtp(i, 0), wtp(i - 1, 2)};
        GTS_TRY(gts_linear_bwd_input_chain_t_f32(g, wt(i, 1), gp, wt(i, 0), h, hbits, g_next, below_t, gm_next, n_rows, fin,
                                                 fout, fin, below_in, packed, stream));
        gm = gm_next, cur ^= 1;
      } else {
        GTS_TRY(igrad(g, w_self, wt(i, 1), fout, gp, w_pool, wt(i, 0), fin, h, hbits, g_next, fin, wtp(i, 1), wtp(i, 0)));
      }
      g = g_next;
    } else if (gx != nullptr) {
      GTS_TRY(igrad(g, w_self, wt(i, 1), fout, gp, w_pool, wt(i, 0), fin, nullptr, nullptr, gx, fin, wtp(i, 1), wtp(i, 0)));
    }
  }
  for (const auto& grp : groups) {
    const int count = static_cast<int>(grp.g.size());
    for (int first = 0; first < count; first += kMaxWgradProblems) {
      const int q = std::min(kMaxWgradProblems, count - first);
      GTS_TRY(gts_linear_bwd_weight_f32(grp.g.data() + first, grp.a.data() + first, grp.gw.data() + first,
                                        grp.gb.data() + first, q, f32(plan.workspace), plan.workspace_bytes, n_rows, grp.n,
                                        grp.k, stream));
    }
  }
  return GTS_OK;
}
```

gnn-tumor-seg_amd/gts/nn.py:

```python
import os

import torch
import torch.nn as nn
import torch.nn.functional as F

from . import dense, ops


class GraphError(RuntimeError):
    """Counterpart of dgl.DGLError for the checks the layers make."""


def _is_relu(fn):
    return fn in (F.relu, torch.relu, torch.nn.functional.relu)


class _SagePoolLayer(torch.autograd.Function):

    @staticmethod
    def forward(ctx, g, h, w_pool, b_pool, w_self, w_neigh, bias, relu_out, need_bwd):
        h = h.contiguous()
        p = dense.linear_fwd(h, w_pool, bias=b_pool, relu=True)
        m, arg = ops.spmm_max_fwd(g, p, want_arg=need_bwd, relu_input=True)
        out = dense.linear_fwd(h, w_self, m, w_neigh, bias=bias, relu=relu_out)
        if need_bwd:
            ctx.g, ctx.relu_out = g, relu_out
            ctx.save_for_backward(h, m, arg, out if relu_out else None, w_pool, w_self, w_neigh)
        return out

    @staticmethod
    def backward(ctx, gout):
        h, m, arg, out, w_pool, w_self, w_neigh = ctx.saved_tensors
        if not ctx.relu_out:
            g = gout.contiguous()
        elif out.shape[1] % 4 == 0 and out.shape[0] > 0:
            g, _ = ops.gat_act_bwd(gout.contiguous(), out, 2, want_bias_grad=False)
        else:
            g = dense.relu_bwd(gout, out)
        need = ctx.needs_input_grad
        gm = dense.linear_bwd_input(g, w_neigh)
        gp = ops.spmm_max_bwd(ctx.g, gm, arg)
        g_ws, g_wn, g_wp, g_bias, g_bp = _pool_layer_weight_grads(g, gp, h, m, w_pool, w_self)
        gh = dense.linear_bwd_input(g, w_self, gp, w_pool) if need[1] else None
        return None, gh, g_wp, g_bp, g_ws, g_wn, g_bias, None, None


class _SageSumLayer(torch.autograd.Function):

    @staticmethod
    def forward(ctx, g, h, w_self, w_neigh, bias, mode, relu_out, need_bwd):
        h = h.contiguous()
        d = g.dev()
        fin, fout = w_neigh.shape[1], w_neigh.shape[0]
        lin_first = fin > fout
        div = d.deg_clamped if mode == "mean" else d.deg_plus1
        src = dense.linear_fwd(h, w_neigh) if lin_first else h
        neigh = ops.spmm_sum_raw(g, src, div_out=div, add_self=(mode == "gcn"))
        last_w = _identity(fout, h.device) if lin_first else w_neigh
        if w_self is not None:
            out = dense.linear_fwd(h, w_self, neigh, last_w, bias=bias, relu=relu_out)
        else:
            out = dense.linear_fwd(neigh, last_w, bias=bias, relu=relu_out)
        if need_bwd:
            ctx.g, ctx.mode, ctx.relu_out, ctx.lin_first = g, mode, relu_out, lin_first
            ctx.has_bias = bias is not None
            ctx.save_for_backward(h, neigh if not lin_first else None, out if relu_out else None, w_self, w_neigh)
        return out

    @staticmethod
    def backward(ctx, gout):
        h, neigh, out, w_self, w_neigh = ctx.saved_tensors
        g, mode = ctx.g, ctx.mode
        d = g.dev()
        div = d.deg_clamped if mode == "mean" else d.deg_plus1
        need = ctx.needs_input_grad
        g_pre, g_bias = ops.gat_act_bwd(gout.contiguous(), out, 2 if ctx.relu_out else 0, want_bias_grad=ctx.has_bias)

        def reduce_bwd(t, accum=None):
            return ops.spmm_sum_raw(g, t, transposed=True, div_in=div, add_self=(mode == "gcn"), accum=accum)

        g_ws = None
        if ctx.lin_first:
            gt = reduce_bwd(g_pre)
            if w_self is not None:
                (g_ws, _), (g_wn, _) = dense.linear_bwd_weight_multi([(g_pre, h, False), (gt, h, False)])
                gh = dense.linear_bwd_input(g_pre, w_self, gt, w_neigh) if need[1] else None
            else:
                g_wn, _ = dense.linear_bwd_weight(gt, h)
                gh = dense.linear_bwd_input(gt, w_neigh) if need[1] else None
        else:
            if w_self is not None:
                (g_ws, _), (g_wn, _) = dense.linear_bwd_weight_multi([(g_pre, h, False), (g_pre, neigh, False)])
            else:
                g_wn, _ = dense.linear_bwd_weight(g_pre, neigh)
            gh = None
            if need[1]:
                gneigh = dense.linear_bwd_input(g_pre, w_neigh)
                gself = dense.linear_bwd_input(g_pre, w_self) if w_self is not None else None
                gh = reduce_bwd(gneigh, accum=gself)
        return None, gh, g_ws, g_wn, g_bias, None, None, None


_identities = {}


def _identity(n, device):
    key = (n, device)
    if key not in _identities:
        _identities[key] = torch.eye(n, dtype=torch.float32, device=device)
    return _identities[key]


OVERLAP_WEIGHT_GRADS = os.environ.get("GTS_OVERLAP_WGRAD", "0") != "0"
TRANSPOSED_IGRAD = os.environ.get("GTS_TRANSPOSED_IGRAD", "1") != "0"
_side_streams = {}


def _side_stream(device):
    s = _side_streams.get(device)
    if s is None:
        try:
            priority = torch.cuda.Stream.priority_range()[0]
        except Exception:
            priority = 0
        s = torch.cuda.Stream(device=device, priority=priority)
        _side_streams[device] = s
    return s


CHAIN_LAYER_GEMMS = os.environ.get("GTS_CHAIN_GEMMS", "1") != "0"
RELU_MASK_BITS = os.environ.get("GTS_RELU_BITS", "1") != "0"


def _chainable(a0, w0, a1, w2):
    n, k0, k1, n2 = w0.shape[0], a0.shape[1], a1.shape[1], w2.shape[0]
    return n % 4 == 0 and k0 % 4 == 0 and k1 % 4 == 0 and n <= 256 and n2 <= 256 and w2.shape[1] == n


def _pool_layer_weight_grads(g, gp, h, m, w_pool, w_self):
    if w_pool.shape == w_self.shape:
        (g_ws, g_bias), (g_wn, _), (g_wp, g_bp) = dense.linear_bwd_weight_multi(
            [(g, h, True), (g, m, False), (gp, h, True)])
    else:
        (g_ws, g_bias), (g_wn, _) = dense.linear_bwd_weight_multi([(g, h, True), (g, m, False)])
        g_wp, g_bp = dense.linear_bwd_weight(gp, h, want_bias_grad=True)
    return g_ws, g_wn, g_wp, g_bias, g_bp


def _pack_by_shape(weights, transposed):
    by_shape, out = {}, {}
    for w in weights:
        by_shape.setdefault(tuple(w.shape), []).append(w)
    for ws in by_shape.values():
        for w, wp in zip(ws, dense.pack_weights(ws, transposed=transposed)):
            out[id(w)] = wp
    return out


class _SagePoolStack(torch.autograd.Function):

    @staticmethod
    def forward(ctx, g, x, need_bwd, *params):
        n_layers = len(params) // 5
        h = x.contiguous()
        saved = []
        hbits = None
        p = None
        fragment = _pack_by_shape([w for i in range(n_layers) for w in (params[5 * i], params[5 * i + 2], params[5 * i + 3])
                                   if w.shape[0] > 128 and w.shape[1] % 4 == 0], transposed=False)
        for i in range(n_layers):
            w_pool, b_pool, w_self, w_neigh, bias = params[5 * i:5 * i + 5]
            last = i == n_layers - 1
            if p is None:
                p = dense.linear_fwd(h, w_pool, bias=b_pool, relu=True, packed=(fragment.get(id(w_pool)), None))
            m, arg = ops.spmm_max_fwd(g, p, want_arg=need_bwd, relu_input=True)
            p = None
            nxt = params[5 * (i + 1):5 * (i + 1) + 2] if not last else None
            obits = dense.relu_bits_empty(h.shape[0], w_self.shape[0], h.device) \
                if RELU_MASK_BITS and need_bwd and not last and dense.relu_bits_pay(h.shape[0], w_self.shape[0]) else None
            if CHAIN_LAYER_GEMMS and nxt is not None and _chainable(h, w_self, m, nxt[0]):
                out, p = dense.linear_fwd_chain(h, w_self, m, w_neigh, bias, True, nxt[0], nxt[1], True, relu_bits=obits,
                                                packed=(fragment.get(id(w_self)), fragment.get(id(w_neigh)), fragment.get(id(nxt[0]))))
            else:
                out = dense.linear_fwd(h, w_self, m, w_neigh, bias=bias, relu=not last, relu_bits=obits,
                                       packed=(fragment.get(id(w_self)), fragment.get(id(w_neigh))))
            saved += [h, m, arg, hbits]
            h, hbits = out, obits
        if need_bwd:
            ctx.g, ctx.n_layers = g, n_layers
            ctx.save_for_backward(*saved, *params)
        return h

    @staticmethod
    def backward(ctx, gout):
        n = ctx.n_layers
        tensors = ctx.saved_tensors
        acts, params = tensors[:4 * n], tensors[4 * n:]
        grads = [None] * (5 * n)
        g = gout.contiguous()
        gx = None
        main = torch.cuda.current_stream()
        side = _side_stream(g.device) if OVERLAP_WEIGHT_GRADS else None
        keep_alive = []
        deferred = {}

        turned, turned_fragment = {}, {}
        if TRANSPOSED_IGRAD:
            by_shape = {}
            for w in (params[5 * i + j] for i in range(n) for j in (0, 2, 3)):
                if w.shape[1] >= 128 and w.shape[0] % 4 == 0 and w.shape[1] % 4 == 0:
                    by_shape.setdefault(tuple(w.shape), []).append(w)
            for ws in by_shape.values():
                plain, packed = dense.pack_weights(ws, transposed=True, want_plain=True)
                for w, wt, wp in zip(ws, plain, packed):
                    turned[id(w)], turned_fragment[id(w)] = wt, wp

        def igrad(g0, w0, g1=None, w1=None, relu_mask=None, relu_bits=None):
            if id(w0) in turned and (w1 is None or id(w1) in turned) and g0.is_contiguous():
                return dense.linear_bwd_input_t(g0, turned[id(w0)], g1, turned[id(w1)] if w1 is not None else None,
                                                relu_mask=relu_mask, relu_bits=relu_bits,
                                                packed=(turned_fragment[id(w0)], turned_fragment[id(w1)] if w1 is not None else None))
            return dense.linear_bwd_input(g0, w0, g1, w1, relu_mask=relu_mask)

        def defer(grad_out, act, slot, bias_slot):
            key = (grad_out.shape[1], act.shape[1])
            deferred.setdefault(key, []).append((grad_out, act, bias_slot is not None, slot, bias_slot))

        gm = None
        for i in reversed(range(n)):
            h, m, arg, hbits = acts[4 * i:4 * i + 4]
            w_pool, _b_pool, w_self, w_neigh, _bias = params[5 * i:5 * i + 5]
            if gm is None:
                gm = igrad(g, w_neigh)
            gp = ops.spmm_max_bwd(ctx.g, gm, arg)
            gm = None
            if side is None:
                defer(gp, h, 5 * i, 5 * i + 1)
                defer(g, h, 5 * i + 2, 5 * i + 4)
                defer(g, m, 5 * i + 3, None)
            else:
                ready = torch.cuda.Event()
                ready.record(main)
                with torch.cuda.stream(side):
                    side.wait_event(ready)
                    g_ws, g_wn, g_wp, g_bias, g_bp = _pool_layer_weight_grads(g, gp, h, m, w_pool, w_self)
                keep_alive.append((g, gp))
                grads[5 * i:5 * i + 5] = [g_wp, g_bp, g_ws, g_wn, g_bias]
            if i > 0:
                below = params[5 * (i - 1) + 3]
                if CHAIN_LAYER_GEMMS and all(id(w) in turned for w in (w_self, w_pool, below)) \
                        and _chainable(g, w_self.t(), gp, below.t()):
                    g, gm = dense.linear_bwd_input_chain_t(g, turned[id(w_self)], gp, turned[id(w_pool)], h,
                                                           turned[id(below)], relu_bits=hbits,
                                                           packed=(turned_fragment[id(w_self)], turned_fragment[id(w_pool)],
                                                                   turned_fragment[id(below)]))
                else:
                    g = igrad(g, w_self, gp, w_pool, relu_mask=h, relu_bits=hbits)
            elif ctx.needs_input_grad[1]:
                gx = igrad(g, w_self, gp, w_pool)
        for problems in deferred.values():
            results = dense.linear_bwd_weight_multi([(go, act, want) for go, act, want, _, _ in problems])
            for (gw, gb), (_, _, _, slot, bias_slot) in zip(results, problems):
                grads[slot] = gw
                if bias_slot is not None:
                    grads[bias_slot] = gb
        if side is not None:
            main.wait_stream(side)
            for t in grads:
                t.record_stream(main)
            for pair in keep_alive:
                for t in pair:
                    t.record_stream(side)
        return (None, gx, None, *grads)


STACK_IN_ONE_CALL = os.environ.get("GTS_STACK_C", "1") != "0"


class GradSink:

    def __init__(self, params, extra=0):
        self.params = list(params)
        self.offsets, at = {}, 0
        for p in self.params:
            self.offsets[id(p)] = at
            at += p.numel()
        self.n, self.extra = at, int(extra)
        self.flat, self.filled = None, False

    def new_buffer(self):
        self.flat = torch.empty(self.n + self.extra, dtype=torch.float32, device=self.params[0].device)
        self.filled = False
        return self.flat


_active_sink = None


class grad_sink:
    def __init__(self, sink):
        self.sink = sink

    def __enter__(self):
        global _active_sink
        self.previous, _active_sink = _active_sink, self.sink
        return self.sink

    def __exit__(self, *exc):
        global _active_sink
        _active_sink = self.previous
        return False


_stack_tables = {}


def _stack_table(params, in_feats):
    import ctypes

    ptrs = [p.data_ptr() for p in params]
    key = (in_feats, *ptrs, *[tuple(p.shape) for p in params])
    hit = _stack_tables.get(key)
    if hit is None:
        n_layers = len(params) // 5
        widths = [in_feats] + [params[5 * i + 2].shape[0] for i in range(n_layers)]
        hit = ((ctypes.c_void_p * (5 * n_layers))(*ptrs), (ctypes.c_int64 * (n_layers + 1))(*widths), widths)
        if len(_stack_tables) > 64:
            _stack_tables.clear()
        _stack_tables[key] = hit
    return hit


def _stack_flags():
    return (1 if CHAIN_LAYER_GEMMS else 0) | (2 if RELU_MASK_BITS else 0) | (4 if TRANSPOSED_IGRAD else 0)


class _SagePoolStackCall(torch.autograd.Function):

    @staticmethod
    def forward(ctx, g, x, need_bwd, *params):
        import ctypes

        from . import _lib
        from ._lib import check, current_stream, ptr

        lib = _lib.load()
        x = x.contiguous()
        n, n_layers = x.shape[0], len(params) // 5
        table, c_widths, widths = _stack_table(params, x.shape[1])
        flags, ab = _stack_flags(), g.arg_bytes
        d = g.dev()
        offsets = (ctypes.c_int64 * (4 * n_layers + 2))()
        total = lib.gts_sage_pool_stack_fwd_arena(n, c_widths, n_layers, 1 if need_bwd else 0, ab, flags, offsets)
        if total < 0:
            raise _lib.GtsError("gts_sage_pool_stack_fwd_arena rejected the stack's shape")
        arena = torch.empty(max(int(total), 16), dtype=torch.uint8, device=x.device)
        ds = ops._cluster_schedule(g, "in", n, 256, ab if need_bwd else 0) if 256 in widths[:-1] else None
        h = ds.host if ds is not None else None
        check(lib.gts_sage_pool_stack_fwd_f32(
            ptr(d.indptr), ptr(d.indices), ptr(ds.packed) if ds else None, h.n_clusters if h else 0,
            h.limits[0] if h else 0, h.limits[1] if h else 0, h.loc_words if h else 0, ptr(x), table, n, c_widths,
            n_layers, 1 if need_bwd else 0, ab, flags, arena.data_ptr(), int(total), current_stream()),
            "gts_sage_pool_stack_fwd_f32")
        at = int(offsets[4 * (n_layers - 1) + 2])
        out = arena[at:at + 4 * n * widths[-1]].view(torch.float32).view(n, widths[-1])
        if need_bwd:
            ctx.g, ctx.widths, ctx.flags, ctx.ab = g, widths, flags, ab
            ctx.param_ids = [id(p) for p in params]
            ctx.save_for_backward(x, arena, *params)
        return out

    @staticmethod
    def backward(ctx, gout):
        import ctypes

        from . import _lib
        from ._lib import check, current_stream, ptr

        lib = _lib.load()
        x, arena, *params = ctx.saved_tensors
        g, widths, flags, ab = ctx.g, ctx.widths, ctx.flags, ctx.ab
        n, n_layers = x.shape[0], len(params) // 5
        gout = gout.contiguous()
        d = g.dev()
        sink = _active_sink
        if sink is not None and (len(ctx.param_ids) != len(sink.params) or
                                 not all(i in sink.offsets for i in ctx.param_ids)):
            sink = None
        sizes = [p.numel() for p in params]
        if sink is not None:
            flat, starts = sink.flat, [sink.offsets[i] for i in ctx.param_ids]
        else:
            flat = torch.empty(sum(sizes), dtype=torch.float32, device=x.device)
            starts = [0] * len(sizes)
            for q in range(1, len(sizes)):
                starts[q] = starts[q - 1] + sizes[q - 1]
        base = flat.data_ptr()
        grads = (ctypes.c_void_p * (5 * n_layers))(*[base + 4 * s for s in starts])
        table, c_widths, _ = _stack_table(params, x.shape[1])
        need = lib.gts_sage_pool_stack_bwd_scratch(n, c_widths, n_layers, flags)
        scratch = torch.empty(max(int(need), 16), dtype=torch.uint8, device=x.device)
        gx = torch.empty_like(x) if ctx.needs_input_grad[1] else None
        ds = ops._cluster_schedule(g, "out", n, 256, ab) if 256 in widths[:-1] else None
        h = ds.host if ds is not None else None
        check(lib.gts_sage_pool_stack_bwd_f32(
            ptr(d.t_indptr), ptr(d.t_indices), ptr(d.t_slot), ptr(ds.packed) if ds else None, h.n_clusters if h else 0,
            h.limits[0] if h else 0, h.limits[1] if h else 0, h.loc_words if h else 0, ptr(gout), ptr(x), table, n,
            c_widths, n_layers, ab, flags, arena.data_ptr(), grads, ptr(gx), scratch.data_ptr(), int(need),
            current_stream()), "gts_sage_pool_stack_bwd_f32")
        if sink is not None:
            sink.filled = True
            return (None, gx, None, *([None] * len(params)))
        return (None, gx, None, *[flat[s:s + k].view_as(p) for s, k, p in zip(starts, sizes, params)])


def sage_pool_stack(graph, features, layers):
    for i, layer in enumerate(layers):
        last = i == len(layers) - 1
        if not isinstance(layer, SAGEConv) or layer._aggre_type != "pool" or layer.bias is None \
                or layer.norm is not None or (layer.feat_drop.p > 0 and layer.training):
            return None
        if (layer.activation is not None) if last else (not _is_relu(layer.activation)):
            return None
    params = []
    for layer in layers:
        params += [layer.fc_pool.weight, layer.fc_pool.bias, layer.fc_self.weight,
                   layer.fc_neigh.weight, layer.bias]
    need_bwd = torch.is_grad_enabled() and (features.requires_grad or any(p.requires_grad for p in params))
    one_call = STACK_IN_ONE_CALL and not ops.INSTRUMENTED and not OVERLAP_WEIGHT_GRADS and features.shape[1] % 4 == 0 \
        and all(p.shape[-1] % 4 == 0 and p.shape[0] % 4 == 0 and p.is_contiguous() for p in params) \
        and features.dtype == torch.float32 and features.is_cuda
    return (_SagePoolStackCall if one_call else _SagePoolStack).apply(graph, features, need_bwd, *params)


class SAGEConv(nn.Module):

    def __init__(self, in_feats, out_feats, aggregator_type, feat_drop=0.0, bias=True, norm=None,
                 activation=None):
        super().__init__()
        if aggregator_type not in ("mean", "gcn", "pool"):
            raise KeyError(f"Invalid aggregator_type. Must be one of mean, gcn, pool. "
                           f"But got {aggregator_type!r} instead.")
        self._in_src_feats = self._in_dst_feats = int(in_feats)
        self._out_feats = int(out_feats)
        self._aggre_type = aggregator_type
        self.norm = norm
        self.feat_drop = nn.Dropout(feat_drop)
        self.activation = activation
        if aggregator_type == "pool":
            self.fc_pool = nn.Linear(in_feats, in_feats)
        if aggregator_type != "gcn":
            self.fc_self = nn.Linear(in_feats, out_feats, bias=False)
        self.fc_neigh = nn.Linear(in_feats, out_feats, bias=False)
        if bias:
            self.bias = nn.Parameter(torch.zeros(out_feats))
        else:
            self.register_buffer("bias", None)
        self.reset_parameters()

    def reset_parameters(self):
        gain = nn.init.calculate_gain("relu")
        if self._aggre_type == "pool":
            nn.init.xavier_uniform_(self.fc_pool.weight, gain=gain)
        if self._aggre_type != "gcn":
            nn.init.xavier_uniform_(self.fc_self.weight, gain=gain)
        nn.init.xavier_uniform_(self.fc_neigh.weight, gain=gain)

    def _load_from_state_dict(self, state_dict, prefix, *args, **kwargs):
        legacy = [prefix + "fc_self.bias", prefix + "fc_neigh.bias"]
        if prefix + "bias" not in state_dict and any(k in state_dict for k in legacy):
            folded = sum(state_dict.pop(k) for k in legacy if k in state_dict)
            state_dict[prefix + "bias"] = folded
        super()._load_from_state_dict(state_dict, prefix, *args, **kwargs)

    def forward(self, graph, feat):
        h = self.feat_drop(feat)
        fused_relu = _is_relu(self.activation)
        if self._aggre_type == "pool":
            bias = self.bias if self.bias is not None else torch.zeros(
                self._out_feats, dtype=h.dtype, device=h.device)
            need_bwd = torch.is_grad_enabled() and (
                h.requires_grad or any(p.requires_grad for p in self.parameters()))
            rst = _SagePoolLayer.apply(graph, h, self.fc_pool.weight, self.fc_pool.bias,
                                       self.fc_self.weight, self.fc_neigh.weight, bias,
                                       fused_relu, need_bwd)
        elif self._out_feats % 4 == 0 and h.shape[0] > 0:
            need_bwd = torch.is_grad_enabled() and (
                h.requires_grad or any(p.requires_grad for p in self.parameters()))
            w_self = self.fc_self.weight if self._aggre_type != "gcn" else None
            rst = _SageSumLayer.apply(graph, h, w_self, self.fc_neigh.weight, self.bias, self._aggre_type,
                                      fused_relu, need_bwd)
        else:
            lin_before_mp = self._in_src_feats > self._out_feats
            src = dense.linear(h, self.fc_neigh.weight) if lin_before_mp else h
            neigh = ops.spmm_reduce(graph, src, self._aggre_type)
            if not lin_before_mp:
                neigh = dense.linear(neigh, self.fc_neigh.weight)
            rst = neigh if self._aggre_type == "gcn" else dense.linear(h, self.fc_self.weight) + neigh
            if self.bias is not None:
                rst = rst + self.bias
            if fused_relu:
                rst = torch.relu(rst)
        if self.activation is not None and not fused_relu:
            rst = self.activation(rst)
        if self.norm is not None:
            rst = self.norm(rst)
        return rst


FUSE_GAT_LAYER = os.environ.get("GTS_FUSE_GAT", "1") != "0"
FUSE_GAT_SCORES = os.environ.get("GTS_FUSE_GAT_SCORES", "1") != "0"


FOLD_GAT_ACT_BWD = os.environ.get("GTS_FOLD_GAT_ACT", "1") != "0"


PACK_GAT_WEIGHTS = os.environ.get("GTS_PACK_GAT", "1") != "0"


def _turn(ws):
    if PACK_GAT_WEIGHTS:
        plain, packed = dense.pack_weights(ws, transposed=True, want_plain=True)
        return plain, tuple(packed) if len(packed) > 1 else (packed[0], None)
    return dense.transpose_batch(ws), (None, None)


class ActLink:
    __slots__ = ("folded", "g_bias", "armed")

    def __init__(self):
        self.folded, self.g_bias, self.armed = False, None, 0


class _GATLayer(torch.autograd.Function):

    @staticmethod
    def forward(ctx, g, h, w_fc, attn_l, attn_r, bias, w_res, identity_res, slope, act_code, heads, dim,
                need_bwd, below=None, above=None):
        h = h.contiguous()
        n = h.shape[0]
        al, ar = attn_l.reshape(heads, dim), attn_r.reshape(heads, dim)
        if FUSE_GAT_SCORES and h.shape[1] % 4 == 0:
            ft, el, er = ops.gat_fc_scores(h, w_fc, al, ar, heads, dim)
        else:
            ft = dense.linear_fwd(h, w_fc).view(n, heads, dim)
            el, er = ops.gat_scores(ft, al, ar)
        if w_res is not None:
            res = dense.linear_fwd(h, w_res)
        elif identity_res:
            res = h
        else:
            res = None
        out, attn = ops._gat_fwd(g, ft, el, er, slope, bias, res, act_code)
        if need_bwd:
            ctx.g, ctx.slope, ctx.act, ctx.identity_res = g, slope, act_code, identity_res
            ctx.save_for_backward(h, ft, el, er, attn, out if act_code else None, w_fc, al, ar, w_res)
            ctx.attn_shape = attn_l.shape
            ctx.below, ctx.above = below, above if act_code == 1 else None
            if ctx.above is not None:
                ctx.above.armed = act_code
        return out

    @staticmethod
    def backward(ctx, gout):
        h, ft, el, er, attn, out, w_fc, al, ar, w_res = ctx.saved_tensors
        n, heads, dim = ft.shape
        need = ctx.needs_input_grad
        if ctx.above is not None and ctx.above.folded:
            g_pre, g_bias = gout.reshape(n, heads * dim), ctx.above.g_bias if need[5] else None
            ctx.above.folded, ctx.above.g_bias, ctx.above.armed = False, None, 0
        else:
            g_pre, g_bias = ops.gat_act_bwd(gout.reshape(n, heads * dim),
                                            out.view(n, heads * dim) if out is not None else None, ctx.act,
                                            want_bias_grad=need[5])
        gft, gel, ger = ops._gat_bwd(ctx.g, ft, el, er, attn, g_pre.view(n, heads, dim), ctx.slope, al, ar)
        g_al, g_ar = ops.gat_param_grad(ft, gel, ger)
        gft2 = gft.view(n, heads * dim)
        g_wres = None
        turn = TRANSPOSED_IGRAD and need[1] and w_fc.shape[1] >= 128 and w_fc.shape[0] % 4 == 0 \
            and w_fc.shape[1] % 4 == 0 and n >= 4096
        fold = turn and ctx.below is not None and ctx.below.armed == 1 and not ctx.identity_res and FOLD_GAT_ACT_BWD
        act_below = ctx.below.armed if fold else 0
        if w_res is not None:
            (g_wfc, _), (g_wres, _) = dense.linear_bwd_weight_multi([(gft2, h, False), (g_pre, h, False)])
            if fold:
                wt, wtp = _turn([w_fc, w_res])
                gh, ctx.below.g_bias = dense.linear_bwd_input_t_act(gft2, wt[0], h, act_below, g_pre, wt[1], packed=wtp)
                ctx.below.folded = True
            elif turn:
                wt, wtp = _turn([w_fc, w_res])
                gh = dense.linear_bwd_input_t(gft2, wt[0], g_pre, wt[1], packed=wtp)
            else:
                gh = dense.linear_bwd_input(gft2, w_fc, g_pre, w_res) if need[1] else None
        else:
            g_wfc, _ = dense.linear_bwd_weight(gft2, h)
            if fold:
                wt, wtp = _turn([w_fc])
                gh, ctx.below.g_bias = dense.linear_bwd_input_t_act(gft2, wt[0], h, act_below, packed=(wtp[0], None))
                ctx.below.folded = True
            elif turn:
                wt, wtp = _turn([w_fc])
                gh = dense.linear_bwd_input_t(gft2, wt[0], packed=(wtp[0], None))
            else:
                gh = dense.linear_bwd_input(gft2, w_fc) if need[1] else None
            if gh is not None and ctx.identity_res:
                gh = gh + g_pre
        return (None, gh, g_wfc, g_al.view(ctx.attn_shape), g_ar.view(ctx.attn_shape), g_bias, g_wres,
                None, None, None, None, None, None, None, None)


class GATConv(nn.Module):

    def __init__(self, in_feats, out_feats, num_heads, feat_drop=0.0, attn_drop=0.0,
                 negative_slope=0.2, residual=False, activation=None,
                 allow_zero_in_degree=False, bias=True):
        super().__init__()
        self._in_feats, self._out_feats, self._num_heads = int(in_feats), int(out_feats), int(num_heads)
        self._allow_zero_in_degree = allow_zero_in_degree
        self.fc = nn.Linear(in_feats, out_feats * num_heads, bias=False)
        self.attn_l = nn.Parameter(torch.empty(1, num_heads, out_feats))
        self.attn_r = nn.Parameter(torch.empty(1, num_heads, out_feats))
        self.feat_drop = nn.Dropout(feat_drop)
        self.attn_drop = nn.Dropout(attn_drop)
        self.negative_slope = negative_slope
        if bias:
            self.bias = nn.Parameter(torch.empty(num_heads * out_feats))
        else:
            self.register_buffer("bias", None)
        if residual:
            if in_feats != out_feats * num_heads:
                self.res_fc = nn.Linear(in_feats, num_heads * out_feats, bias=False)
            else:
                self.res_fc = nn.Identity()
        else:
            self.register_buffer("res_fc", None)
        self.activation = activation
        self.reset_parameters()

    def reset_parameters(self):
        gain = nn.init.calculate_gain("relu")
        nn.init.xavier_normal_(self.fc.weight, gain=gain)
        nn.init.xavier_normal_(self.attn_l, gain=gain)
        nn.init.xavier_normal_(self.attn_r, gain=gain)
        if self.bias is not None:
            nn.init.constant_(self.bias, 0)
        if isinstance(self.res_fc, nn.Linear):
            nn.init.xavier_normal_(self.res_fc.weight, gain=gain)

    def forward(self, graph, feat, below=None, above=None):
        if not self._allow_zero_in_degree and graph.min_in_degree == 0:
            raise GraphError(
                "There are 0-in-degree nodes in the graph, output for those nodes will be invalid. "
                "Adding self-loop on the input graph resolves the issue; setting "
                "allow_zero_in_degree=True suppresses the check.")
        if self.attn_drop.p > 0 and self.training:
            raise NotImplementedError("attention dropout is not built (the reference never sets it: "
                                      "model/networks.py:77-78 passes no dropout to GAT)")
        n = feat.shape[0]
        h = self.feat_drop(feat)
        if above is not None:
            above.armed = 0
        act_code = 0 if self.activation is None else 1 if self.activation in (F.elu, torch.nn.functional.elu) else -1
        if FUSE_GAT_LAYER and act_code >= 0 and self._out_feats % 4 == 0 and feat.dim() == 2:
            w_res = self.res_fc.weight if isinstance(self.res_fc, nn.Linear) else None
            identity_res = isinstance(self.res_fc, nn.Identity)
            need_bwd = torch.is_grad_enabled() and (
                h.requires_grad or any(p.requires_grad for p in self.parameters()))
            if self.feat_drop.p > 0 and self.training:
                below = None
            return _GATLayer.apply(graph, h, self.fc.weight, self.attn_l, self.attn_r, self.bias, w_res,
                                   identity_res, self.negative_slope, act_code, self._num_heads,
                                   self._out_feats, need_bwd, below, above)
        ft = dense.linear(h, self.fc.weight).view(n, self._num_heads, self._out_feats)
        el = (ft * self.attn_l).sum(dim=-1)
        er = (ft * self.attn_r).sum(dim=-1)
        rst = ops.gat_aggregate(graph, ft, el, er, self.negative_slope)
        if self.res_fc is not None:
            res = dense.linear(h, self.res_fc.weight) if isinstance(self.res_fc, nn.Linear) else h
            rst = rst + res.view(n, -1, self._out_feats)
        if self.bias is not None:
            rst = rst + self.bias.view(1, self._num_heads, self._out_feats)
        if self.activation is not None:
            rst = self.activation(rst)
        return rst
```

gnn-tumor-seg_amd/gts/ops.py:

```python
import torch

from . import _lib
from ._lib import check, current_stream, ptr, require_device

_ARG_DTYPE = {0: torch.uint8, 1: torch.uint8, 4: torch.int32}

KERNEL_TIMERS = {}
INSTRUMENTED = False


def _timed(name, launch):
    timer = KERNEL_TIMERS.get(name)
    return timer(launch) if timer is not None else launch()


def _expect(tensor, shape, name):
    if tensor is not None and tuple(tensor.shape) != tuple(shape):
        raise _lib.GtsError(f"{name}: expected shape {tuple(shape)}, got {tuple(tensor.shape)}")


def _f32(*tensors):
    for t in tensors:
        if t is not None and t.dtype != torch.float32:
            raise _lib.GtsError(f"gts kernels are fp32: got {t.dtype}")


_cluster_counters = {}


def cluster_counters(device):
    key = (device, current_stream())
    buf = _cluster_counters.get(key)
    if buf is None:
        buf = torch.zeros(256, dtype=torch.int32, device=device)
        _cluster_counters[key] = buf
    return buf


def spmm_max_fwd(g, x, want_arg=True, relu_input=False):
    x = x.contiguous()
    _f32(x)
    require_device(x)
    d = g.dev()
    if x.dim() != 2 or x.shape[0] != g.n:
        raise _lib.GtsError(f"features must be [graph nodes = {g.n}, F], got {tuple(x.shape)}")
    n, f = g.n, x.shape[1]
    out = torch.empty((n, f), dtype=torch.float32, device=x.device)
    ab = g.arg_bytes if want_arg else 0
    arg = torch.empty((n, f), dtype=_ARG_DTYPE[ab], device=x.device) if want_arg else None
    lib = _lib.load()
    ds = _cluster_schedule(g, "in", n, f, ab)
    if ds is not None:
        h = ds.host

        def launch():
            return lib.gts_spmm_max_fwd_cluster_f32(ptr(ds.packed), h.n_clusters, h.limits[0], h.limits[1], h.loc_words,
                                                    ptr(x), ptr(out), ptr(arg), ab, 1 if relu_input else 0, n, f,
                                                    ptr(cluster_counters(x.device)), current_stream())
    else:
        def launch():
            return lib.gts_spmm_max_fwd_f32(ptr(d.indptr), ptr(d.indices), ptr(x), ptr(out), ptr(arg),
                                            ab, 1 if relu_input else 0, n, f, current_stream())

    code = _timed("spmm_max_fwd_f256", launch) if (f == 256 and want_arg) else launch()
    check(code, "gts_spmm_max_fwd_f32")
    return out, arg


def _cluster_schedule(g, which, n, f, arg_bytes):
    from . import schedule

    if not schedule.ENABLED or f != 256 or arg_bytes not in (0, 1) or n * 1024 >= 2 ** 32 or n == 0:
        return None
    if which == "in" and n < schedule.MIN_ROWS_FORWARD:
        return None
    return g.dev_schedule(which)


def spmm_max_bwd(g, gout, arg, relu_src=None):
    gout = gout.contiguous()
    _f32(gout, relu_src)
    require_device(gout, arg, relu_src)
    d = g.dev()
    if gout.dim() != 2 or gout.shape[0] != g.n:
        raise _lib.GtsError(f"gradient must be [graph nodes = {g.n}, F], got {tuple(gout.shape)}")
    n, f = g.n, gout.shape[1]
    _expect(arg, (n, f), "arg")
    _expect(relu_src, (n, f), "relu_src")
    if arg.dtype != _ARG_DTYPE[g.arg_bytes]:
        raise _lib.GtsError(f"arg dtype {arg.dtype} does not belong to this graph ({_ARG_DTYPE[g.arg_bytes]})")
    gx = torch.empty((n, f), dtype=torch.float32, device=gout.device)
    lib = _lib.load()
    ds = _cluster_schedule(g, "out", n, f, arg.element_size()) if relu_src is None else None
    if ds is not None:
        h = ds.host

        def launch():
            return lib.gts_spmm_max_bwd_cluster_f32(ptr(ds.packed), h.n_clusters, h.limits[0], h.limits[1], h.loc_words,
                                                    ptr(gout), ptr(arg), 1, ptr(gx), n, f, ptr(cluster_counters(gout.device)),
                                                    current_stream())
    else:
        def launch():
            return lib.gts_spmm_max_bwd_f32(ptr(d.t_indptr), ptr(d.t_indices), ptr(d.t_slot), ptr(gout),
                                            ptr(arg), arg.element_size(), ptr(relu_src), ptr(gx), n, f,
                                            current_stream())

    check(_timed("spmm_max_bwd_f256", launch) if f == 256 else launch(), "gts_spmm_max_bwd_f32")
    return gx


def spmm_sum_raw(g, x, transposed=False, div_in=None, div_out=None, add_self=False, accum=None):
    x = x.contiguous()
    _f32(x, div_in, div_out, accum)
    require_device(x, div_in, div_out, accum)
    d = g.dev()
    indptr, indices = (d.t_indptr, d.t_indices) if transposed else (d.indptr, d.indices)
    n = g.n
    if x.dim() != 2 or x.shape[0] != n:
        raise _lib.GtsError(f"features must be [graph nodes = {n}, F], got {tuple(x.shape)}")
    f = x.shape[1]
    _expect(div_in, (n,), "div_in")
    _expect(div_out, (n,), "div_out")
    _expect(accum, (n, f), "accum")
    out = torch.empty_like(x)
    check(_lib.load().gts_spmm_sum_f32(ptr(indptr), ptr(indices), ptr(x), ptr(out), ptr(div_in), ptr(div_out),
                                       ptr(accum), 1 if add_self else 0, n, f, current_stream()), "gts_spmm_sum_f32")
    return out


class _SpMMMax(torch.autograd.Function):
    @staticmethod
    def forward(ctx, g, x):
        out, arg = spmm_max_fwd(g, x, want_arg=True)
        ctx.g = g
        ctx.save_for_backward(arg)
        return out

    @staticmethod
    def backward(ctx, gout):
        (arg,) = ctx.saved_tensors
        return None, spmm_max_bwd(ctx.g, gout, arg)


class _SpMMReduce(torch.autograd.Function):

    @staticmethod
    def forward(ctx, g, x, mode):
        ctx.g, ctx.mode = g, mode
        d = g.dev()
        if mode == "sum":
            return spmm_sum_raw(g, x)
        if mode == "mean":
            return spmm_sum_raw(g, x, div_out=d.deg_clamped)
        if mode == "gcn":
            return spmm_sum_raw(g, x, div_out=d.deg_plus1, add_self=True)
        raise ValueError(mode)

    @staticmethod
    def backward(ctx, gout):
        g, mode = ctx.g, ctx.mode
        d = g.dev()
        if mode == "sum":
            gx = spmm_sum_raw(g, gout, transposed=True)
        elif mode == "mean":
            gx = spmm_sum_raw(g, gout, transposed=True, div_in=d.deg_clamped)
        else:
            gx = spmm_sum_raw(g, gout, transposed=True, div_in=d.deg_plus1, add_self=True)
        return None, gx, None


def spmm_max(g, x):
    return _SpMMMax.apply(g, x)


def spmm_reduce(g, x, mode):
    return _SpMMReduce.apply(g, x, mode)


def _gat_fwd(g, ft, el, er, slope, bias=None, residual=None, activation=0):
    d = g.dev()
    if ft.dim() != 3 or ft.shape[0] != g.n:
        raise _lib.GtsError(f"ft must be [graph nodes = {g.n}, H, D], got {tuple(ft.shape)}")
    n, h, dim = ft.shape
    _expect(el, (n, h), "el")
    _expect(er, (n, h), "er")
    _expect(bias, (h * dim,), "bias")
    if residual is not None and (residual.shape[0] != n or residual.numel() != n * h * dim):
        raise _lib.GtsError(f"residual must hold [{n}, {h}*{dim}] values, got {tuple(residual.shape)}")
    out = torch.empty_like(ft)
    attn = torch.empty((g.number_of_edges(), h), dtype=torch.float32, device=ft.device)
    lib = _lib.load()
    ds = _gat_cluster_schedule(g, "gat_in", n, h, dim) if residual is None else None
    if ds is not None:
        hs = ds.host
        nbytes = lib.gts_gat_cluster_workspace(hs.n_clusters, hs.limits[0], hs.loc_words, h, 0)
        ws = _gat_ws(ft.device, nbytes)
        launch = lambda: lib.gts_gat_fwd_cluster_f32(
            ptr(d.indptr), ptr(d.indices), ptr(ds.packed), hs.n_clusters, hs.limits[0], hs.limits[1], hs.loc_words,
            1 if hs.tagged else 0, ptr(ft), ptr(el), ptr(er), float(slope), ptr(bias), activation, ptr(out), ptr(attn),
            ptr(ws), nbytes, n, h, dim, g.max_in_degree, current_stream())
    else:
        launch = lambda: lib.gts_gat_fwd_f32(
            ptr(d.indptr), ptr(d.indices), ptr(ft), ptr(el), ptr(er), float(slope), ptr(bias), ptr(residual),
            activation, ptr(out), ptr(attn), n, h, dim, current_stream())
    check(_timed("gat_fwd", launch) if h * dim >= 256 else launch(), "gts_gat_fwd_f32")
    return out, attn


_gat_workspaces = {}


def _gat_ws(device, nbytes):
    key = (device, current_stream())
    buf = _gat_workspaces.get(key)
    if buf is None or buf.numel() * 4 < nbytes:
        buf = torch.empty((nbytes + 3) // 4, dtype=torch.float32, device=device)
        _gat_workspaces[key] = buf
    return buf


def _gat_cluster_schedule(g, which, n, heads, dim):
    from . import schedule

    if not schedule.ENABLED_GAT or dim != 256 or n < schedule.MIN_ROWS_GAT or n * heads * 1024 >= 2 ** 32 or heads > 64:
        return None
    if which.endswith("in") and g.max_in_degree > 64:
        return None
    return g.dev_schedule(which)


def _gat_bwd(g, ft, el, er, attn, gout, slope, attn_l=None, attn_r=None):
    d = g.dev()
    if ft.dim() != 3 or ft.shape[0] != g.n:
        raise _lib.GtsError(f"ft must be [graph nodes = {g.n}, H, D], got {tuple(ft.shape)}")
    n, h, dim = ft.shape
    _expect(el, (n, h), "el")
    _expect(er, (n, h), "er")
    _expect(attn, (g.number_of_edges(), h), "attn")
    _expect(gout, (n, h, dim), "gout")
    _expect(attn_l, (h, dim), "attn_l")
    _expect(attn_r, (h, dim), "attn_r")
    lib = _lib.load()
    ge = torch.empty_like(attn)
    ger = torch.empty_like(er)
    wide = h * dim >= 256
    es = _gat_cluster_schedule(g, "gat_edge_in", n, h, dim) if g.max_in_degree <= 8 else None
    if es is not None:
        hs = es.host
        nbytes = 2 * lib.gts_gat_cluster_workspace(hs.n_clusters, hs.limits[0], hs.loc_words, h, 0)
        ws_e = _gat_ws(ft.device, nbytes)
        edge = lambda: lib.gts_gat_bwd_edge_cluster_f32(
            ptr(d.indptr), ptr(d.indices), ptr(es.packed), hs.n_clusters, hs.limits[0], hs.limits[1], hs.loc_words,
            1 if hs.tagged else 0, ptr(ft), ptr(el), ptr(er), ptr(attn), ptr(gout), float(slope), ptr(ge), ptr(ger),
            ptr(ws_e), nbytes, n, h, dim, g.max_in_degree, current_stream())
    else:
        edge = lambda: lib.gts_gat_bwd_edge_f32(ptr(d.indptr), ptr(d.indices), ptr(ft), ptr(el), ptr(er), ptr(attn),
                                                ptr(gout), float(slope), ptr(ge), ptr(ger), n, h, dim, current_stream())
    check(_timed("gat_bwd_edge", edge) if wide else edge(), "gts_gat_bwd_edge_f32")
    gft = torch.empty_like(ft)
    gel = torch.empty_like(el)
    ds = _gat_cluster_schedule(g, "gat_out", n, h, dim)
    if ds is not None:
        hs = ds.host
        nbytes = lib.gts_gat_cluster_workspace(hs.n_clusters, hs.limits[0], hs.loc_words, h, 1)
        ws = _gat_ws(ft.device, nbytes)
        attn_lr = torch.stack([attn_l.reshape(-1), attn_r.reshape(-1)]) if attn_l is not None else None
        src = lambda: lib.gts_gat_bwd_src_cluster_f32(
            ptr(d.t_indptr), ptr(d.t_pos), ptr(ds.packed), hs.n_clusters, hs.limits[0], hs.limits[1], hs.loc_words,
            1 if hs.tagged else 0, ptr(attn), ptr(ge), ptr(gout), ptr(attn_lr), ptr(ger) if attn_l is not None else None,
            ptr(gft), ptr(gel), ptr(ws), nbytes, n, h, dim, g.max_out_degree, current_stream())
    else:
        src = lambda: lib.gts_gat_bwd_src_f32(ptr(d.t_indptr), ptr(d.t_indices), ptr(d.t_pos), ptr(attn), ptr(ge),
                                              ptr(gout), ptr(attn_l), ptr(attn_r),
                                              ptr(ger) if attn_l is not None else None, ptr(gft), ptr(gel), n, h, dim,
                                              current_stream())
    check(_timed("gat_bwd_src", src) if wide else src(), "gts_gat_bwd_src_f32")
    return gft, gel, ger


class _GATAggregate(torch.autograd.Function):

    @staticmethod
    def forward(ctx, g, ft, el, er, negative_slope):
        ft, el, er = ft.contiguous(), el.contiguous(), er.contiguous()
        _f32(ft, el, er)
        require_device(ft, el, er)
        out, attn = _gat_fwd(g, ft, el, er, negative_slope)
        ctx.g, ctx.slope = g, float(negative_slope)
        ctx.save_for_backward(ft, el, er, attn)
        return out

    @staticmethod
    def backward(ctx, gout):
        ft, el, er, attn = ctx.saved_tensors
        gft, gel, ger = _gat_bwd(ctx.g, ft, el, er, attn, gout.contiguous(), ctx.slope)
        return None, gft, gel, ger, None


def gat_aggregate(g, ft, el, er, negative_slope):
    return _GATAggregate.apply(g, ft, el, er, negative_slope)


def gat_scores(ft, attn_l, attn_r):
    ft, attn_l, attn_r = ft.contiguous(), attn_l.contiguous(), attn_r.contiguous()
    _f32(ft, attn_l, attn_r)
    require_device(ft, attn_l, attn_r)
    if ft.dim() != 3:
        raise _lib.GtsError(f"ft must be [N, H, D], got {tuple(ft.shape)}")
    n, h, dim = ft.shape
    attn_l, attn_r = attn_l.reshape(-1, dim), attn_r.reshape(-1, dim)
    _expect(attn_l, (h, dim), "attn_l")
    _expect(attn_r, (h, dim), "attn_r")
    el = torch.empty((n, h), dtype=torch.float32, device=ft.device)
    er = torch.empty_like(el)
    check(_lib.load().gts_gat_scores_f32(ptr(ft), ptr(attn_l), ptr(attn_r), ptr(el), ptr(er), n, h, dim,
                                         current_stream()), "gts_gat_scores_f32")
    return el, er


def gat_fc_scores(h, w_fc, attn_l, attn_r, heads, dim, packed=None):
    h, w_fc = h.contiguous(), w_fc.contiguous()
    attn_l, attn_r = attn_l.reshape(heads, dim).contiguous(), attn_r.reshape(heads, dim).contiguous()
    _f32(h, w_fc, attn_l, attn_r)
    require_device(h, w_fc, attn_l, attn_r)
    n, k = h.shape
    if w_fc.dim() != 2 or w_fc.shape[1] != k:
        raise _lib.GtsError(f"shapes do not match: inner dims of h @ fc.weight^T ({k} vs {tuple(w_fc.shape)[-1]})")
    if w_fc.shape[0] != heads * dim:
        raise _lib.GtsError(f"shapes do not match: fc.weight rows ({w_fc.shape[0]}) vs heads * out_feats ({heads * dim})")
    if k % 4:
        raise _lib.GtsError("gat_fc_scores needs an input width that is a multiple of 4")
    lib = _lib.load()
    ft = torch.empty((n, heads, dim), dtype=torch.float32, device=h.device)
    el = torch.empty((n, heads), dtype=torch.float32, device=h.device)
    er = torch.empty_like(el)
    nbytes = lib.gts_gat_fc_scores_workspace(n, heads, dim)
    ws = torch.empty(max(1, nbytes // 4), dtype=torch.float32, device=h.device)
    from . import dense
    if packed is not None:
        dense._packed_array((packed,), (w_fc,))
    dense._timed("fwd", 2.0 * n * heads * dim * k, lambda: check(lib.gts_gat_fc_scores_f32(
        ptr(h), ptr(w_fc), ptr(attn_l), ptr(attn_r), ptr(ft), ptr(el), ptr(er), ptr(ws), ws.numel() * 4, n, heads, dim, k,
        ptr(packed), current_stream()), "gts_gat_fc_scores_f32"))
    return ft, el, er


def _reduce_ws(n, cols, device):
    nbytes = _lib.load().gts_gat_reduce_workspace(n, cols)
    return torch.empty(max(1, nbytes // 4), dtype=torch.float32, device=device)


def gat_act_bwd(gout, out, activation, want_bias_grad):
    gout = gout.contiguous()
    n, cols = gout.shape[0], gout[0].numel()
    if activation:
        _expect(out, gout.shape, "out")
    g_pre = torch.empty_like(gout) if activation else gout
    g_bias = torch.empty(cols, dtype=torch.float32, device=gout.device) if want_bias_grad else None
    ws = _reduce_ws(n, cols, gout.device) if want_bias_grad else None
    check(_lib.load().gts_gat_act_bwd_f32(ptr(gout), ptr(out), activation, ptr(g_pre) if activation else None,
                                          ptr(g_bias), ptr(ws), ws.numel() * 4 if ws is not None else 0,
                                          n, cols, current_stream()), "gts_gat_act_bwd_f32")
    return g_pre, g_bias


def gat_param_grad(ft, gel, ger):
    n, h, dim = ft.shape
    _expect(gel, (n, h), "gel")
    _expect(ger, (n, h), "ger")
    gl = torch.empty((h, dim), dtype=torch.float32, device=ft.device)
    gr = torch.empty_like(gl)
    ws = _reduce_ws(n, h * dim, ft.device)
    check(_lib.load().gts_gat_param_grad_f32(ptr(ft), ptr(gel), ptr(ger), ptr(gl), ptr(gr), ptr(ws),
                                             ws.numel() * 4, n, h, dim, current_stream()),
          "gts_gat_param_grad_f32")
    return gl, gr


def project_rows(svs, table, bg_row):
    if svs.dtype != torch.int16:
        raise _lib.GtsError("supervoxel partitioning must be int16 (mri2graph/graphgen.py:77)")
    svs = svs.contiguous()
    table = table.contiguous()
    bg_row = bg_row.to(table.dtype).contiguous()
    require_device(svs, table, bg_row)
    row_bytes = table.element_size() * (table[0].numel() if table.shape[0] else bg_row.numel())
    if bg_row.numel() * bg_row.element_size() != row_bytes:
        raise _lib.GtsError("background row does not match table rows")
    out = torch.empty(tuple(svs.shape) + tuple(table.shape[1:]), dtype=table.dtype, device=svs.device)
    if svs.numel() == 0:
        return out
    lib = _lib.load()
    check(_timed("project_rows", lambda: lib.gts_project_rows_i16(
        ptr(svs), ptr(table), ptr(bg_row), ptr(out), svs.numel(), table.shape[0], row_bytes,
        current_stream())), "gts_project_rows_i16")
    return out


def project_argmax(svs, logits, relabel=None):
    _f32(logits)
    if svs.dtype != torch.int16:
        raise _lib.GtsError("supervoxel partitioning must be int16")
    svs, logits = svs.contiguous(), logits.contiguous()
    require_device(svs, logits, relabel)
    if relabel is not None and (relabel.dtype != torch.int16 or relabel.numel() < logits.shape[1]):
        raise _lib.GtsError("relabel must be int16 with one entry per class")
    out = torch.empty(svs.shape, dtype=torch.int16, device=svs.device)
    if svs.numel() == 0:
        return out
    check(_lib.load().gts_project_argmax_i16(ptr(svs), ptr(logits), ptr(relabel), ptr(out), svs.numel(),
                                             logits.shape[0], logits.shape[1], current_stream()),
          "gts_project_argmax_i16")
    return out


def project_argmax_occupancy(svs, logits):
    _f32(logits)
    if svs.dtype != torch.int16 or svs.dim() != 3:
        raise _lib.GtsError("supervoxel partitioning must be a 3-D int16 volume")
    svs, logits = svs.contiguous(), logits.contiguous()
    require_device(svs, logits)
    dx, dy, dz = svs.shape
    out = torch.empty(svs.shape, dtype=torch.int16, device=svs.device)
    occ = torch.zeros(dx + dy + dz, dtype=torch.uint8, device=svs.device)
    if svs.numel():
        check(_lib.load().gts_project_argmax_occupancy_i16(ptr(svs), ptr(logits), ptr(out), ptr(occ), dx, dy, dz,
                                                           logits.shape[0], logits.shape[1], current_stream()),
              "gts_project_argmax_occupancy_i16")
    return out, (occ[:dx], occ[dx:dx + dy], occ[dx + dy:])


class CropBox:

    def __init__(self, xs, ys, zs, volume_shape, device):
        import numpy as np

        self.volume_shape = tuple(int(d) for d in volume_shape)
        self.host = []
        for idx, extent in zip((xs, ys, zs), self.volume_shape):
            idx = np.asarray(idx).reshape(-1).astype(np.int64)
            if idx.size and (idx.min() < 0 or idx.max() >= extent or np.any(np.diff(idx) <= 0)):
                raise _lib.GtsError("crop indices must be strictly ascending and inside the volume")
            self.host.append(idx)
        self.shape = tuple(len(i) for i in self.host)
        self.dev = [torch.from_numpy(i.astype(np.int32)).to(device) for i in self.host]

    def as_ix(self):
        import numpy as np

        return np.ix_(*self.host)


def crop_concat(img, svs, table, bg_row, box):
    _f32(img, table, bg_row)
    if svs.dtype != torch.int16 or tuple(svs.shape) != box.volume_shape:
        raise _lib.GtsError("partitioning must be int16 with the crop box's volume shape")
    ci = 0
    if img is not None:
        if img.dim() != 4 or tuple(img.shape[:3]) != box.volume_shape:
            raise _lib.GtsError("image must be [X, Y, Z, C] over the same volume")
        img, ci = img.contiguous(), img.shape[3]
    svs, table, bg_row = svs.contiguous(), table.contiguous(), bg_row.contiguous()
    require_device(svs, table, bg_row, img, *box.dev)
    ct = table.shape[1]
    if bg_row.numel() != ct:
        raise _lib.GtsError("background row does not match table rows")
    cx, cy, cz = box.shape
    out = torch.empty((1, ci + ct, cx, cy, cz), dtype=torch.float32, device=svs.device)
    if out.numel():
        check(_lib.load().gts_crop_concat_f32(ptr(img), ptr(svs), ptr(table), ptr(bg_row), ptr(box.dev[0]),
                                              ptr(box.dev[1]), ptr(box.dev[2]), ptr(out), cx, cy, cz,
                                              box.volume_shape[1], box.volume_shape[2], table.shape[0], ci, ct,
                                              current_stream()), "gts_crop_concat_f32")
    return out


def argmax_scatter(scores, box, relabel=None):
    _f32(scores)
    if scores.dim() == 5 and scores.shape[0] == 1:
        scores = scores[0]
    if scores.dim() != 4 or tuple(scores.shape[1:]) != box.shape:
        raise _lib.GtsError("scores must be [C, cx, cy, cz] over the crop box")
    scores = scores.contiguous()
    require_device(scores, relabel, *box.dev)
    if relabel is not None and (relabel.dtype != torch.int16 or relabel.numel() < scores.shape[0]):
        raise _lib.GtsError("relabel must be int16 with one entry per class")
    out = torch.zeros(box.volume_shape, dtype=torch.int16, device=scores.device)
    cx, cy, cz = box.shape
    if scores.numel():
        check(_lib.load().gts_argmax_scatter_i16(ptr(scores), ptr(relabel), ptr(box.dev[0]), ptr(box.dev[1]),
                                                 ptr(box.dev[2]), ptr(out), cx, cy, cz, box.volume_shape[1],
                                                 box.volume_shape[2], scores.shape[0], current_stream()),
              "gts_argmax_scatter_i16")
    return out


def label_confusion(pred, truth):
    if pred.dtype != torch.int16 or truth.dtype != torch.int16:
        raise _lib.GtsError("label_confusion takes int16 labels")
    if pred.numel() != truth.numel():
        raise _lib.GtsError(f"label_confusion: {pred.numel()} predictions vs {truth.numel()} labels")
    pred, truth = pred.contiguous(), truth.contiguous()
    require_device(pred, truth)
    counts = torch.zeros((5, 5), dtype=torch.int64, device=pred.device)
    if pred.numel():
        lib = _lib.load()
        scratch = torch.empty(lib.gts_label_confusion_workspace(pred.numel()), dtype=torch.uint8,
                              device=pred.device)
        check(lib.gts_label_confusion_i16(ptr(pred), ptr(truth), ptr(counts), ptr(scratch), scratch.numel(),
                                          pred.numel(), current_stream()), "gts_label_confusion_i16")
    return counts


class _WeightedCE(torch.autograd.Function):

    @staticmethod
    def forward(ctx, logits, labels, class_w):
        logits, labels = logits.contiguous(), labels.contiguous()
        _f32(logits, class_w)
        require_device(logits, labels, class_w)
        if logits.dim() != 2 or labels.dtype != torch.int64 or labels.shape != logits.shape[:1]:
            raise _lib.GtsError("weighted CE takes logits [N, C] and int64 labels [N]")
        n, c = logits.shape
        _expect(class_w, (c,), "class_w")
        lib = _lib.load()
        ws = torch.empty(max(1, lib.gts_weighted_ce_workspace(n) // 4), dtype=torch.float32, device=logits.device)
        grad = torch.empty_like(logits) if ctx.needs_input_grad[0] else None
        stats = torch.empty(3, dtype=torch.float32, device=logits.device)
        check(lib.gts_weighted_ce_f32(ptr(logits), ptr(labels), ptr(class_w), ptr(grad), ptr(ws), ws.numel() * 4,
                                      ptr(stats), n, c, current_stream()), "gts_weighted_ce_f32")
        ctx.save_for_backward(grad, stats)
        ctx.mark_non_differentiable(stats)
        ctx.set_materialize_grads(False)
        return stats[2].clone(), stats[0].clone(), stats

    @staticmethod
    def backward(ctx, g_mean, g_sum, _g_stats):
        grad_unscaled, stats = ctx.saved_tensors
        if g_mean is None and g_sum is None:
            return None, None, None
        if g_sum is None:
            scale = g_mean / stats[1]
        elif g_mean is None:
            scale = g_sum
        else:
            scale = g_sum + g_mean / stats[1]
        return grad_unscaled * scale, None, None


def weighted_cross_entropy(logits, labels, class_w=None, reduction="mean"):
    mean, total, _ = _WeightedCE.apply(logits, labels, class_w)
    if reduction == "mean":
        return mean
    if reduction == "sum":
        return total
    raise ValueError(reduction)


def weighted_ce_numerator_grad(logits, labels, class_w=None):
    logits_c, labels = logits.detach().contiguous(), labels.contiguous()
    _f32(logits_c, class_w)
    require_device(logits_c, labels, class_w)
    if logits_c.dim() != 2 or labels.dtype != torch.int64 or labels.shape != logits_c.shape[:1]:
        raise _lib.GtsError("weighted CE takes logits [N, C] and int64 labels [N]")
    n, c = logits_c.shape
    _expect(class_w, (c,), "class_w")
    lib = _lib.load()
    ws = torch.empty(max(1, lib.gts_weighted_ce_workspace(n) // 4), dtype=torch.float32, device=logits_c.device)
    grad = torch.empty_like(logits_c)
    stats = torch.empty(3, dtype=torch.float32, device=logits_c.device)
    check(lib.gts_weighted_ce_f32(ptr(logits_c), ptr(labels), ptr(class_w), ptr(grad), ptr(ws), ws.numel() * 4,
                                  ptr(stats), n, c, current_stream()), "gts_weighted_ce_f32")
    return grad, stats


def weighted_cross_entropy_stats(logits, labels, class_w=None):
    _, total, stats = _WeightedCE.apply(logits, labels, class_w)
    return total, stats
```

include/gts_hip.h:

```cpp
#ifndef GTS_HIP_H
#define GTS_HIP_H

#include <stdint.h>

#ifdef __cplusplus
extern "C" {
#endif

#define GTS_OK 0
#define GTS_ERR_NULL (-1)
#define GTS_ERR_SHAPE (-2)
#define GTS_ERR_ARGKIND (-3)

int32_t gts_abi_version(void);
const char* gts_error_string(int32_t code);

int32_t gts_spmm_max_fwd_f32(const int32_t* indptr, const int32_t* indices, const float* x,
                             float* out, void* arg, int32_t arg_bytes, int32_t relu_input,
                             int64_t n_dst, int64_t n_feat, void* stream);

int32_t gts_spmm_max_bwd_f32(const int32_t* t_indptr, const int32_t* t_indices,
                             const int32_t* t_slot, const float* gout, const void* arg,
                             int32_t arg_bytes, const float* relu_src, float* gx,
                             int64_t n_src, int64_t n_feat, void* stream);

int64_t gts_cluster_record_words(int32_t max_rows, int32_t max_srcs, int32_t loc_words, int32_t with_tag);
int32_t gts_cluster_schedule(const int32_t* indptr, const int32_t* indices, const int32_t* t_indptr,
                             const int32_t* t_indices, const int32_t* edge_tag, int64_t n_rows,
                             int32_t max_rows, int32_t max_srcs, int32_t max_edges, int32_t* rec,
                             int64_t rec_capacity, int64_t* n_clusters, int64_t* n_staged,
                             int32_t* max_cluster_edges);
int64_t gts_cluster_lds_bytes(int32_t max_rows, int32_t max_srcs, int32_t loc_words, int32_t kind);
int32_t gts_spmm_max_fwd_cluster_f32(const int32_t* rec, int64_t n_clusters, int32_t max_rows, int32_t max_srcs,
                                     int32_t loc_words, const float* x, float* out, void* arg,
                                     int32_t arg_bytes, int32_t relu_input, int64_t n_rows, int64_t n_feat,
                                     uint32_t* counters, void* stream);
int32_t gts_spmm_max_bwd_cluster_f32(const int32_t* rec, int64_t n_clusters, int32_t max_rows, int32_t max_srcs,
                                     int32_t loc_words, const float* gout, const void* arg, int32_t arg_bytes,
                                     float* gx, int64_t n_rows, int64_t n_feat, uint32_t* counters, void* stream);
#define GTS_CLUSTER_COUNTER_WORDS 256
int32_t gts_cluster_uses_counters(int64_t n_clusters, int32_t max_rows, int32_t max_srcs, int32_t loc_words, int32_t backward);

int32_t gts_spmm_sum_f32(const int32_t* indptr, const int32_t* indices, const float* x,
                         float* out, const float* div_in, const float* div_out, const float* accum,
                         int32_t add_self, int64_t n_out, int64_t n_feat, void* stream);

int32_t gts_gat_fwd_f32(const int32_t* indptr, const int32_t* indices, const float* ft,
                        const float* el, const float* er, float negative_slope, const float* bias,
                        const float* residual, int32_t activation, float* out, float* attn,
                        int64_t n, int64_t heads, int64_t dim, void* stream);
int32_t gts_gat_scores_f32(const float* ft, const float* attn_l, const float* attn_r, float* el,
                           float* er, int64_t n, int64_t heads, int64_t dim, void* stream);

int32_t gts_gat_bwd_edge_f32(const int32_t* indptr, const int32_t* indices, const float* ft,
                             const float* el, const float* er, const float* attn,
                             const float* gout, float negative_slope, float* ge, float* ger,
                             int64_t n, int64_t heads, int64_t dim, void* stream);
int32_t gts_gat_bwd_src_f32(const int32_t* t_indptr, const int32_t* t_indices,
                            const int32_t* t_pos, const float* attn, const float* ge,
                            const float* gout, const float* attn_l, const float* attn_r,
                            const float* ger, float* gft, float* gel, int64_t n, int64_t heads,
                            int64_t dim, void* stream);
int64_t gts_gat_reduce_workspace(int64_t n, int64_t cols);
int32_t gts_gat_act_bwd_f32(const float* gout, const float* out, int32_t activation, float* g_pre,
                            float* g_bias, float* workspace, int64_t workspace_bytes, int64_t n,
                            int64_t cols, void* stream);
int32_t gts_gat_param_grad_f32(const float* ft, const float* gel, const float* ger, float* g_attn_l,
                               float* g_attn_r, float* workspace, int64_t workspace_bytes, int64_t n,
                               int64_t heads, int64_t dim, void* stream);

int64_t gts_gat_cluster_workspace(int64_t n_clusters, int32_t max_rows, int32_t loc_words, int64_t heads, int32_t backward);
int32_t gts_gat_attn_f32(const int32_t* indptr, const int32_t* indices, const float* el, const float* er,
                         float negative_slope, float* attn, int64_t n, int64_t heads, int64_t max_degree, void* stream);
int32_t gts_gat_fwd_cluster_f32(const int32_t* indptr, const int32_t* indices, const int32_t* rec, int64_t n_clusters,
                                int32_t max_rows, int32_t max_srcs, int32_t loc_words, int32_t tagged, const float* ft,
                                const float* el, const float* er, float negative_slope, const float* bias,
                                int32_t activation, float* out, float* attn, float* workspace, int64_t workspace_bytes,
                                int64_t n, int64_t heads, int64_t dim, int64_t max_degree, void* stream);
int32_t gts_gat_bwd_edge_cluster_f32(const int32_t* indptr, const int32_t* indices, const int32_t* rec, int64_t n_clusters,
                                     int32_t max_rows, int32_t max_srcs, int32_t loc_words, int32_t tagged, const float* ft,
                                     const float* el, const float* er, const float* attn, const float* gout,
                                     float negative_slope, float* ge, float* ger, float* workspace, int64_t workspace_bytes,
                                     int64_t n, int64_t heads, int64_t dim, int64_t max_degree, void* stream);
int32_t gts_gat_bwd_src_cluster_f32(const int32_t* t_indptr, const int32_t* t_pos, const int32_t* rec, int64_t n_clusters,
                                    int32_t max_rows, int32_t max_srcs, int32_t loc_words, int32_t tagged,
                                    const float* attn, const float* ge, const float* gout, const float* attn_lr,
                                    const float* ger, float* gft, float* gel, float* workspace, int64_t workspace_bytes,
                                    int64_t n, int64_t heads, int64_t dim, int64_t max_degree, void* stream);

int32_t gts_project_rows_i16(const int16_t* svs, const void* table, const void* bg_row,
                             void* out, int64_t n_vox, int64_t n_rows, int32_t row_bytes,
                             void* stream);
int32_t gts_project_argmax_i16(const int16_t* svs, const float* logits, const int16_t* relabel,
                               int16_t* out, int64_t n_vox, int64_t n_rows, int64_t n_classes,
                               void* stream);

int32_t gts_project_argmax_occupancy_i16(const int16_t* svs, const float* logits, int16_t* out,
                                         uint8_t* occupancy, int64_t dim_x, int64_t dim_y,
                                         int64_t dim_z, int64_t n_rows, int64_t n_classes,
                                         void* stream);

int32_t gts_crop_concat_f32(const float* img, const int16_t* svs, const float* table,
                            const float* bg_row, const int32_t* xs, const int32_t* ys,
                            const int32_t* zs, float* out, int64_t cx, int64_t cy, int64_t cz,
                            int64_t dim_y, int64_t dim_z, int64_t n_rows, int64_t img_channels,
                            int64_t row_channels, void* stream);
int32_t gts_argmax_scatter_i16(const float* scores, const int16_t* relabel, const int32_t* xs,
                               const int32_t* ys, const int32_t* zs, int16_t* out, int64_t cx,
                               int64_t cy, int64_t cz, int64_t dim_y, int64_t dim_z,
                               int64_t n_classes, void* stream);

int32_t gts_adamw_f32(float* param, const float* grad, float* exp_avg, float* exp_avg_sq, int64_t n,
                      double lr, double beta1, double beta2, double eps, double weight_decay,
                      int64_t step, void* stream);

int64_t gts_label_confusion_workspace(int64_t n);
int32_t gts_label_confusion_i16(const int16_t* pred, const int16_t* truth, int64_t* counts,
                                void* workspace, int64_t workspace_bytes, int64_t n, void* stream);

int64_t gts_relu_bits_bytes(int64_t m, int64_t n);
int32_t gts_relu_bits_pay(int64_t m, int64_t n);
int32_t gts_linear_fwd_f32(const float* a0, const float* w0, const float* a1, const float* w1,
                           const float* bias, float* out, int64_t m, int64_t n, int64_t k0,
                           int64_t k1, int32_t relu, uint64_t* relu_bits, const float* const* packed,
                           void* stream);
int64_t gts_packed_weight_floats(int64_t n, int64_t k);
int32_t gts_pack_weights_f32(const float* const* src, float* const* dst, float* const* plain_t, int32_t n_mats,
                             int64_t rows, int64_t cols, int32_t transposed, void* stream);
int32_t gts_linear_bwd_input_f32(const float* g0, const float* w0, const float* g1, const float* w1,
                                 const float* relu_mask, float* gin, int64_t m, int64_t k,
                                 int64_t n0, int64_t n1, void* stream);
int32_t gts_linear_bwd_input_t_f32(const float* g0, const float* w0t, const float* g1, const float* w1t,
                                   const float* relu_mask, const uint64_t* relu_bits, float* gin, int64_t m,
                                   int64_t k, int64_t n0, int64_t n1, const float* const* packed, void* stream);
int64_t gts_linear_bwd_input_t_act_workspace(int64_t m, int64_t k);
int32_t gts_linear_bwd_input_t_act_f32(const float* g0, const float* w0t, const float* g1, const float* w1t,
                                       const float* act_out, int32_t activation, float* gin, float* g_bias,
                                       float* workspace, int64_t workspace_bytes, int64_t m, int64_t k,
                                       int64_t n0, int64_t n1, const float* const* packed,
                                       void* stream);
int64_t gts_gat_fc_scores_workspace(int64_t m, int64_t heads, int64_t dim);
int32_t gts_gat_fc_scores_f32(const float* h, const float* w_fc, const float* attn_l, const float* attn_r,
                              float* ft, float* el, float* er, float* workspace, int64_t workspace_bytes,
                              int64_t m, int64_t heads, int64_t dim, int64_t k, const float* w_fc_packed, void* stream);
int32_t gts_linear_fwd_chain_f32(const float* a0, const float* w0, const float* a1, const float* w1,
                                 const float* bias, float* out, const float* w2, const float* bias2,
                                 float* out2, int64_t m, int64_t n, int64_t k0, int64_t k1, int32_t relu,
                                 int64_t n2, int32_t relu2, uint64_t* relu_bits, const float* const* packed,
                                 void* stream);
int32_t gts_linear_bwd_input_chain_t_f32(const float* g0, const float* w0t, const float* g1,
                                         const float* w1t, const float* relu_mask, const uint64_t* relu_bits,
                                         float* gin, const float* w2t, float* gin2, int64_t m, int64_t k,
                                         int64_t n0, int64_t n1, int64_t k2, const float* const* packed,
                                         void* stream);
int32_t gts_transpose_batch_f32(const float* const* src, float* const* dst, int32_t n_mats,
                                int64_t rows, int64_t cols, void* stream);
int64_t gts_linear_bwd_weight_workspace(int64_t m, int64_t n, int64_t k, int32_t n_problems);
int32_t gts_linear_bwd_weight_f32(const float* const* g, const float* const* a, float* const* gw,
                                  float* const* gb, int32_t n_problems, float* workspace,
                                  int64_t workspace_bytes, int64_t m, int64_t n, int64_t k,
                                  void* stream);

int64_t gts_sage_pool_stack_fwd_arena(int64_t n_rows, const int64_t* widths, int32_t n_layers, int32_t training,
                                      int32_t arg_bytes, int32_t flags, int64_t* offsets);
int32_t gts_sage_pool_stack_fwd_f32(const int32_t* indptr, const int32_t* indices, const int32_t* sched_rec,
                                    int64_t sched_clusters, int32_t sched_rows, int32_t sched_srcs,
                                    int32_t sched_loc_words, const float* x, const float* const* params,
                                    int64_t n_rows, const int64_t* widths, int32_t n_layers, int32_t training,
                                    int32_t arg_bytes, int32_t flags, void* arena, int64_t arena_bytes, void* stream);
int64_t gts_sage_pool_stack_bwd_scratch(int64_t n_rows, const int64_t* widths, int32_t n_layers, int32_t flags);
int32_t gts_sage_pool_stack_bwd_f32(const int32_t* t_indptr, const int32_t* t_indices, const int32_t* t_slot,
                                    const int32_t* sched_rec, int64_t sched_clusters, int32_t sched_rows,
                                    int32_t sched_srcs, int32_t sched_loc_words, const float* gout, const float* x,
                                    const float* const* params, int64_t n_rows, const int64_t* widths,
                                    int32_t n_layers, int32_t arg_bytes, int32_t flags, const void* fwd_arena,
                                    float* const* grads, float* gx, void* scratch, int64_t scratch_bytes,
                                    void* stream);

int64_t gts_weighted_ce_workspace(int64_t n);
int32_t gts_weighted_ce_f32(const float* logits, const int64_t* labels, const float* class_w,
                            float* grad_unscaled, float* workspace, int64_t workspace_bytes,
                            float* out3, int64_t n, int64_t n_classes, void* stream);

#define GTS_OPT_GEMM_TILE 1
#define GTS_OPT_WGRAD_TILE 2
#define GTS_OPT_IGRAD_TILE 3
#define GTS_OPT_PROJECT_STREAMING 6
#define GTS_OPT_SPMM_ROWS_PER_WAVE 4
#define GTS_OPT_SPMM_STREAMING 5
#define GTS_OPT_GEMM_SCHED 7
#define GTS_OPT_CLUSTER_STREAMING 8
#define GTS_OPT_GAT_WALK 14
#define GTS_OPT_GAT_CLUSTER_WAVES 15
#define GTS_OPT_GAT_CLUSTER_GROUP 16
#define GTS_OPT_GAT_CLUSTER_DEALING 17
#define GTS_OPT_CLUSTER_DEALING 18
#define GTS_OPT_PANEL_ROWS 13
#define GTS_OPT_CLUSTER_RING 10
#define GTS_OPT_CLUSTER_PER_CU 11
#define GTS_OPT_CLUSTER_CONSUMERS 12
int32_t gts_set_option(int32_t option, int32_t value);
int32_t gts_get_option(int32_t option);

#define GTS_COLLATE_MAX_SCHEDULES 6
typedef struct {
  int64_t n_nodes, n_edges;
  const int32_t *indptr, *indices, *t_indptr, *t_indices, *t_slot, *t_pos;
  const void* features;
  const void* labels;
  int32_t feat_bytes;
  int32_t label_bytes;
  const int32_t* sched_rec[GTS_COLLATE_MAX_SCHEDULES];
  int64_t sched_clusters[GTS_COLLATE_MAX_SCHEDULES];
  int32_t sched_loc_words[GTS_COLLATE_MAX_SCHEDULES];
} gts_collate_member_t;
typedef struct {
  int32_t max_rows, max_srcs, tagged, reserved;
} gts_collate_kind_t;
typedef struct {
  int64_t total_bytes, n_nodes, n_edges;
  int64_t features, labels;
  int64_t csr[8];
  int64_t sched[GTS_COLLATE_MAX_SCHEDULES];
  int64_t sched_clusters[GTS_COLLATE_MAX_SCHEDULES];
  int32_t sched_loc_words[GTS_COLLATE_MAX_SCHEDULES];
  int32_t sched_record_words[GTS_COLLATE_MAX_SCHEDULES];
} gts_collate_plan_t;
int32_t gts_collate_plan(const gts_collate_member_t* members, int32_t n_members, int64_t feat_width,
                         const gts_collate_kind_t* kinds, int32_t n_kinds, gts_collate_plan_t* plan);
int32_t gts_collate_batch(const gts_collate_member_t* members, int32_t n_members, int64_t feat_width,
                          const gts_collate_kind_t* kinds, int32_t n_kinds, void* dst, int64_t dst_bytes,
                          int32_t n_threads, gts_collate_plan_t* plan);

#define GTS_GG_MAX_SV 32767
#define GTS_GG_MAX_K 32
#define GTS_GG_MAX_RADIUS 16
int32_t gts_gg_gaussian_f64(const double* in, double* out, double* tmp, const double* weights, int32_t radius,
                            double scale, int64_t d, int64_t h, int64_t w, int64_t c, void* stream);
int32_t gts_gg_slic_assign_f64(const double* img, const double* centres, int32_t n_centres, int64_t d, int64_t h,
                               int64_t w, int64_t c, int32_t step_z, int32_t step_y, int32_t step_x,
                               double spatial_weight, int32_t* labels, uint64_t* best, uint32_t* winner,
                               void* stream);
int32_t gts_gg_slic_update_f64(const double* img, const int32_t* labels, double* centres, int32_t n_centres,
                               int64_t d, int64_t h, int64_t w, int64_t c, int32_t* bbox, void* stream);
int32_t gts_gg_enforce_connectivity(const int32_t* labels, int32_t* out, int64_t d, int64_t h, int64_t w,
                                    int64_t min_size, int64_t max_size, int64_t* queue, int32_t* n_labels);
int64_t gts_gg_sv_stats_workspace(int64_t n_vox, int32_t n_sv);
int32_t gts_gg_sv_stats(const int32_t* partition, const float* intensities, const int16_t* vox_labels, int64_t d,
                        int64_t h, int64_t w, int64_t c, int32_t n_sv, double* feats, double* centroids,
                        int32_t* sv_labels, void* scratch, void* stream);
int32_t gts_gg_discard_f64(const double* feats, const double* centroids, const int32_t* sv_labels, int32_t n_sv,
                           int32_t n_feat, const int32_t* partition, int64_t n_vox, int32_t* remap, int32_t* keep,
                           double* node_feats, double* node_centroids, int32_t* node_labels, int16_t* new_partition,
                           int32_t* n_nodes, void* stream);
int32_t gts_gg_knn_candidates_f64(const double* positions, int32_t n, int32_t k, int32_t* cand, void* stream);
int32_t gts_gg_knn_greedy(const int32_t* cand, int32_t n, int32_t k, int32_t* picks, int32_t* got, int64_t* n_edges);
int64_t gts_gg_touching_workspace(int32_t n);
int32_t gts_gg_touching_count_i16(const int16_t* partition, int64_t d, int64_t h, int64_t w, int32_t n, void* scratch,
                                  int32_t* indptr, void* stream);
int32_t gts_gg_touching_emit(const void* scratch, int32_t n, const int32_t* indptr, int32_t* cols, void* stream);

#ifdef __cplusplus
}
#endif
#endif
```

Baseline: 957.3.

## Store max-pool argmax winners as 4-bit nibbles when in-degree fits

```diff
diff --git a/gnn-tumor-seg_amd/csrc/gts_rows.h b/gnn-tumor-seg_amd/csrc/gts_rows.h
--- a/gnn-tumor-seg_amd/csrc/gts_rows.h
+++ b/gnn-tumor-seg_amd/csrc/gts_rows.h
@@ -33,6 +33,18 @@
   const v2f arg = x * v2f{kLog2e, kLog2e};
   const v2f large = v2f{__builtin_amdgcn_exp2f(arg.x), __builtin_amdgcn_exp2f(arg.y)} - v2f{1.0f, 1.0f};
   return v2f{x.x < kEluSplit ? large.x : small.x, x.y < kEluSplit ? large.y : small.y};
+}
+
+__device__ __forceinline__ uint32_t pack_nibbles(const int (&slot)[4]) {
+  return (slot[0] & 0xF) | ((slot[1] & 0xF) << 4) | ((slot[2] & 0xF) << 8) | ((slot[3] & 0xF) << 12);
+}
+__device__ __forceinline__ int nibble_at(uint32_t w, int t) { return (w >> (4 * t)) & 0xF; }
+__device__ __forceinline__ uint4 octet_nibbles(uint32_t w16) {
+  const uint32_t a = w16 | (static_cast<uint32_t>(__shfl_xor(static_cast<int>(w16), 1)) << 16);
+  const uint32_t b = static_cast<uint32_t>(__shfl_xor(static_cast<int>(a), 2));
+  const uint32_t c = static_cast<uint32_t>(__shfl_xor(static_cast<int>(a), 4));
+  const uint32_t d = static_cast<uint32_t>(__shfl_xor(static_cast<int>(b), 4));
+  return make_uint4(a, b, c, d);
 }
 
 template <int LPR>
diff --git a/gnn-tumor-seg_amd/csrc/gts_spmm.hip b/gnn-tumor-seg_amd/csrc/gts_spmm.hip
--- a/gnn-tumor-seg_amd/csrc/gts_spmm.hip
+++ b/gnn-tumor-seg_amd/csrc/gts_spmm.hip
@@ -50,6 +50,10 @@
     } else {
       slot[0] = p[0];
     }
+  } else if constexpr (ARGB == GTS_ARG_NIBBLE) {
+    const uint32_t w = *(static_cast<const uint16_t*>(arg) + off / 4);
+#pragma unroll
+    for (int t = 0; t < VEC; ++t) slot[t] = nibble_at(w, t);
   } else {
     const int32_t* p = static_cast<const int32_t*>(arg) + off;
     if constexpr (VEC == 4) {
@@ -102,7 +106,16 @@
       const size_t off = static_cast<size_t>(v) * n_feat + c;
       if (active) {
         if (nt & 1) o.store_nt(out + off); else o.store(out + off);
-        if constexpr (ARGB != 0) store_slots<VEC, ARGB>(arg, off, slot);
+        if constexpr (ARGB == 1 || ARGB == 4) store_slots<VEC, ARGB>(arg, off, slot);
+      }
+      if constexpr (ARGB == GTS_ARG_NIBBLE) {
+        const uint32_t w16 = pack_nibbles(slot);
+        if (LPR >= 8 && n_feat % 32 == 0) {
+          const uint4 w = octet_nibbles(w16);
+          if (active && (threadIdx.x & 7) == 0) *reinterpret_cast<uint4*>(static_cast<uint8_t*>(arg) + off / 2) = w;
+        } else if (active) {
+          *(static_cast<uint16_t*>(arg) + off / 4) = static_cast<uint16_t>(w16);
+        }
       }
     });
   }
@@ -223,7 +236,8 @@
   using namespace gts;
   if (!indptr || !x || !out || (arg_bytes != 0 && !arg)) return GTS_ERR_NULL;
   if (bad_shape(n_dst, n_feat)) return GTS_ERR_SHAPE;
-  if (arg_bytes != 0 && arg_bytes != 1 && arg_bytes != 4) return GTS_ERR_ARGKIND;
+  if (arg_bytes != 0 && arg_bytes != 1 && arg_bytes != 4 && arg_bytes != GTS_ARG_NIBBLE) return GTS_ERR_ARGKIND;
+  if (arg_bytes == GTS_ARG_NIBBLE && n_feat % 4 != 0) return GTS_ERR_ARGKIND;
   if (n_dst == 0) return GTS_OK;
   const Geometry g = make_geometry(n_dst, n_feat, 2);
   const int nt = g_spmm_nt < 0 ? 1 : g_spmm_nt;
@@ -234,7 +248,10 @@
       spmm_max_fwd_kernel<VEC, LPR, 0><<<g.grid, kBlock, 0, st>>>(indptr, indices, x, out, arg, nd, nf, g.seq, nt, relu_input);
     else if (arg_bytes == 1)
       spmm_max_fwd_kernel<VEC, LPR, 1><<<g.grid, kBlock, 0, st>>>(indptr, indices, x, out, arg, nd, nf, g.seq, nt, relu_input);
-    else
+    else if (arg_bytes == GTS_ARG_NIBBLE) {
+      if constexpr (VEC == 4)
+        spmm_max_fwd_kernel<VEC, LPR, GTS_ARG_NIBBLE><<<g.grid, kBlock, 0, st>>>(indptr, indices, x, out, arg, nd, nf, g.seq, nt, relu_input);
+    } else
       spmm_max_fwd_kernel<VEC, LPR, 4><<<g.grid, kBlock, 0, st>>>(indptr, indices, x, out, arg, nd, nf, g.seq, nt, relu_input);
   })
   return launch_status();
@@ -248,7 +265,8 @@
   using namespace gts;
   if (!t_indptr || !gout || !arg || !gx) return GTS_ERR_NULL;
   if (bad_shape(n_src, n_feat)) return GTS_ERR_SHAPE;
-  if (arg_bytes != 1 && arg_bytes != 4) return GTS_ERR_ARGKIND;
+  if (arg_bytes != 1 && arg_bytes != 4 && arg_bytes != GTS_ARG_NIBBLE) return GTS_ERR_ARGKIND;
+  if (arg_bytes == GTS_ARG_NIBBLE && n_feat % 4 != 0) return GTS_ERR_ARGKIND;
   if (n_src == 0) return GTS_OK;
   const Geometry g = make_geometry(n_src, n_feat, 1);
   const int nt = g_spmm_nt < 0 ? 0 : g_spmm_nt;
@@ -257,7 +275,10 @@
   GTS_DISPATCH_GEOM(g, {
     if (arg_bytes == 1)
       spmm_max_bwd_kernel<VEC, LPR, 1><<<g.grid, kBlock, 0, st>>>(t_indptr, t_indices, t_slot, gout, arg, relu_src, gx, ns, nf, g.seq, nt);
-    else
+    else if (arg_bytes == GTS_ARG_NIBBLE) {
+      if constexpr (VEC == 4)
+        spmm_max_bwd_kernel<VEC, LPR, GTS_ARG_NIBBLE><<<g.grid, kBlock, 0, st>>>(t_indptr, t_indices, t_slot, gout, arg, relu_src, gx, ns, nf, g.seq, nt);
+    } else
       spmm_max_bwd_kernel<VEC, LPR, 4><<<g.grid, kBlock, 0, st>>>(t_indptr, t_indices, t_slot, gout, arg, relu_src, gx, ns, nf, g.seq, nt);
   })
   return launch_status();
diff --git a/gnn-tumor-seg_amd/csrc/gts_spmm_cluster.hip b/gnn-tumor-seg_amd/csrc/gts_spmm_cluster.hip
--- a/gnn-tumor-seg_amd/csrc/gts_spmm_cluster.hip
+++ b/gnn-tumor-seg_amd/csrc/gts_spmm_cluster.hip
@@ -95,10 +95,27 @@
         *reinterpret_cast<uint32_t*>(a.arg + off) = w;
       }
     }
-  }
-  return trips * (ARGB == 1 ? 2 : 1);
-}
-
+    if constexpr (ARGB == GTS_ARG_NIBBLE && WHATIF != 3) {
+      if (have) {
+        const size_t off = static_cast<size_t>(l_rec[a.layout.rows + j]) * kF + part * (kF / 2) + hl * 4;
+        *reinterpret_cast<uint16_t*>(a.arg + off / 2) = static_cast<uint16_t>(pack_nibbles(slot));
+      }
+    }
+  }
+  return trips * (ARGB != 0 ? 2 : 1);
+}
+
+template <int ARGB>
+__device__ __forceinline__ uint32_t winner_word(const unsigned char* my_w, unsigned s) {
+  if constexpr (ARGB == GTS_ARG_NIBBLE) return *reinterpret_cast<const uint16_t*>(my_w + s * (kArgHalfBytes / 2));
+  else return *reinterpret_cast<const uint32_t*>(my_w + s * kArgHalfBytes);
+}
+template <int ARGB>
+__device__ __forceinline__ unsigned winner_of(uint32_t w, int t) {
+  if constexpr (ARGB == GTS_ARG_NIBBLE) return (w >> (4 * t)) & 0xF;
+  else return (w >> (8 * t)) & 0xFF;
+}
+template <int ARGB>
 __device__ __forceinline__ int reduce_winner_rows(const ClusterArgs& a, const int32_t* l_rec, const unsigned char* image,
                                                   const unsigned char* winners, int part, int first, int step) {
   const int lane = threadIdx.x & (kWave - 1), half = lane >> 5, hl = lane & 31;
@@ -107,7 +124,7 @@
   const uint2* loc = reinterpret_cast<const uint2*>(l_rec + a.layout.loc);
   const uint2* tag = reinterpret_cast<const uint2*>(l_rec + a.layout.tag);
   const unsigned char* my_g = image + hl * 16;
-  const unsigned char* my_w = winners + hl * 4;
+  const unsigned char* my_w = winners + hl * (ARGB == GTS_ARG_NIBBLE ? 2 : 4);
   int trips = 0;
   for (int j0 = 2 * first; j0 < n_rows; j0 += 2 * step, ++trips) {
     const int j = j0 + half;
@@ -131,15 +148,15 @@
             for (int q = 0; q < N; ++q) {
               const unsigned s = chunk_byte(w, Q0 + q);
               g[q] = *reinterpret_cast<const float4*>(my_g + s * kHalfBytes);
-              win[q] = *reinterpret_cast<const uint32_t*>(my_w + s * kArgHalfBytes);
+              win[q] = winner_word<ARGB>(my_w, s);
             }
 #pragma unroll
             for (int q = 0; q < N; ++q) {
               const unsigned want = chunk_byte(tg, Q0 + q);
-              acc[0] += (win[q] & 0xFF) == want ? g[q].x : 0.0f;
-              acc[1] += ((win[q] >> 8) & 0xFF) == want ? g[q].y : 0.0f;
-              acc[2] += ((win[q] >> 16) & 0xFF) == want ? g[q].z : 0.0f;
-              acc[3] += (win[q] >> 24) == want ? g[q].w : 0.0f;
+              acc[0] += winner_of<ARGB>(win[q], 0) == want ? g[q].x : 0.0f;
+              acc[1] += winner_of<ARGB>(win[q], 1) == want ? g[q].y : 0.0f;
+              acc[2] += winner_of<ARGB>(win[q], 2) == want ? g[q].z : 0.0f;
+              acc[3] += winner_of<ARGB>(win[q], 3) == want ? g[q].w : 0.0f;
             }
           };
           group(IC<0>{}, IC<FIRST>{});
@@ -161,7 +178,7 @@
             for (int q = 0; q < N; ++q) {
               const unsigned s = chunk_byte(w, Q0 + q);
               g[q] = *reinterpret_cast<const float4*>(my_g + s * kHalfBytes);
-              win[q] = *reinterpret_cast<const uint32_t*>(my_w + s * kArgHalfBytes);
+              win[q] = winner_word<ARGB>(my_w, s);
             }
 #pragma unroll
             for (int q = 0; q < N; ++q) {
@@ -169,7 +186,7 @@
               const bool live = 8 * c + Q0 + q < deg;
               const float g4[4] = {g[q].x, g[q].y, g[q].z, g[q].w};
 #pragma unroll
-              for (int t = 0; t < 4; ++t) acc[t] += (live && ((win[q] >> (8 * t)) & 0xFF) == want) ? g4[t] : 0.0f;
+              for (int t = 0; t < 4; ++t) acc[t] += (live && winner_of<ARGB>(win[q], t) == want) ? g4[t] : 0.0f;
             }
           };
           group(IC<0>{}, IC<FIRST>{});
@@ -186,14 +203,19 @@
   return trips;
 }
 
-template <typename Dma, typename SrcOf>
+template <int ARGB>
+constexpr int kWinHalfBytes = ARGB == GTS_ARG_NIBBLE ? kArgHalfBytes / 2 : kArgHalfBytes;
+template <int ARGB>
+constexpr int kWinRowsPerDma = 1024 / kWinHalfBytes<ARGB>;
+template <int ARGB, typename Dma, typename SrcOf>
 __device__ __forceinline__ void gather_winner_halves(const Dma& dma, int part, unsigned char* image,
                                                      int n_srcs, int first, int step, SrcOf&& src_of) {
-  const int l8 = threadIdx.x & 7;
+  constexpr int kLanes = kWinHalfBytes<ARGB> / 16;
+  const int lr = threadIdx.x & (kLanes - 1);
   for (int i = first; i < n_srcs; i += step) {
-    const unsigned voff = static_cast<unsigned>(src_of(i)) * static_cast<unsigned>(kF) +
-                          static_cast<unsigned>(part) * kArgHalfBytes + l8 * 16u;
-    dma(image + i * kArgHalfBytes, voff);
+    const unsigned voff = static_cast<unsigned>(src_of(i)) * static_cast<unsigned>(2 * kWinHalfBytes<ARGB>) +
+                          static_cast<unsigned>(part) * kWinHalfBytes<ARGB> + lr * 16u;
+    dma(image + i * kWinHalfBytes<ARGB>, voff);
   }
 }
 
@@ -274,14 +296,15 @@
       return half ? s1 : s0;
     });
     if constexpr (BWD) {
-      const int32_t ids8 = l_rec[a.layout.srcs + min(8 * (wave + n_waves * (lane >> 3)) + (lane & 7), last)];
-      int k8 = 0;
-      gather_winner_halves(rw, part, image + ((a.max_srcs + 1) & ~1) * kHalfBytes, n_srcs, 8 * wave, 8 * n_waves, [&](int) {
-        const int32_t id = __builtin_amdgcn_ds_bpermute(4 * (8 * k8 + (lane >> 3)), ids8);
-        ++k8;
+      constexpr int R = kWinRowsPerDma<ARGB>;
+      const int32_t ids_r = l_rec[a.layout.srcs + min(R * (wave + n_waves * (lane / R)) + (lane % R), last)];
+      int kr = 0;
+      gather_winner_halves<ARGB>(rw, part, image + ((a.max_srcs + 1) & ~1) * kHalfBytes, n_srcs, R * wave, R * n_waves, [&](int) {
+        const int32_t id = __builtin_amdgcn_ds_bpermute(4 * (R * kr + lane / (kWave / R)), ids_r);
+        ++kr;
         return id;
       });
-      return k + k8;
+      return k + kr;
     }
     return k;
   };
@@ -349,7 +372,7 @@
       stores = WHATIF == 3 ? (reduce_max_rows<ARGB, WHATIF>(a, l_rec, image, part, wave, n_waves), 0)
                            : reduce_max_rows<ARGB, WHATIF>(a, l_rec, image, part, wave, n_waves);
     else if constexpr (BWD)
-      stores = reduce_winner_rows(a, l_rec, image, image + ((a.max_srcs + 1) & ~1) * kHalfBytes, part, wave, n_waves);
+      stores = reduce_winner_rows<ARGB>(a, l_rec, image, image + ((a.max_srcs + 1) & ~1) * kHalfBytes, part, wave, n_waves);
     else
       stores = reduce_max_rows<ARGB>(a, l_rec, image, part, wave, n_waves);
     lap(3);
@@ -373,13 +396,15 @@
 struct LdsPlan {
   int slot_bytes, image_off, win_off;
 };
-inline LdsPlan lds_plan(int max_rows, int max_srcs, int loc_words, bool bwd) {
+inline LdsPlan lds_plan(int max_rows, int max_srcs, int loc_words, bool bwd, int argb = 1) {
   const RecLayout l = rec_layout(max_rows, max_srcs, loc_words, bwd);
   LdsPlan p;
   p.image_off = (l.words * 4 + 15) & ~15;
   const int image = ((max_srcs + 1) & ~1) * kHalfBytes;
   p.win_off = p.image_off + image;
-  p.slot_bytes = p.win_off + (bwd ? ((max_srcs + 7) & ~7) * kArgHalfBytes : 0);
+  const int win_rows = argb == GTS_ARG_NIBBLE ? kWinRowsPerDma<GTS_ARG_NIBBLE> : kWinRowsPerDma<1>;
+  const int win_bytes = argb == GTS_ARG_NIBBLE ? kWinHalfBytes<GTS_ARG_NIBBLE> : kWinHalfBytes<1>;
+  p.slot_bytes = p.win_off + (bwd ? (max_srcs + win_rows - 1) / win_rows * win_rows * win_bytes : 0);
   return p;
 }
 
@@ -405,7 +430,7 @@
 
 template <bool BWD, int ARGB, int WHATIF = 0>
 inline int launch_cluster(ClusterArgs a, int max_rows, int loc_words, hipStream_t st) {
-  const LdsPlan p = lds_plan(max_rows, a.max_srcs, loc_words, BWD);
+  const LdsPlan p = lds_plan(max_rows, a.max_srcs, loc_words, BWD, ARGB);
   a.image_off = p.image_off, a.win_off = p.win_off, a.slot_bytes = p.slot_bytes;
   if (p.slot_bytes > kMaxLds) return GTS_ERR_SHAPE;
   const int64_t units = 2LL * a.n_clusters;
@@ -590,8 +615,8 @@
 }
 
 extern "C" int64_t gts_cluster_lds_bytes(int32_t max_rows, int32_t max_srcs, int32_t loc_words, int32_t kind) {
-  if (max_rows < 1 || max_srcs < 1 || loc_words < 0 || loc_words % 4 != 0 || (kind != 0 && kind != 1)) return -1;
-  return gts::lds_plan(max_rows, max_srcs, loc_words, kind == 1).slot_bytes;
+  if (max_rows < 1 || max_srcs < 1 || loc_words < 0 || loc_words % 4 != 0 || kind < 0 || kind > 2) return -1;
+  return gts::lds_plan(max_rows, max_srcs, loc_words, kind != 0, kind == 2 ? GTS_ARG_NIBBLE : 1).slot_bytes;
 }
 
 namespace {
@@ -607,7 +632,7 @@
 extern "C" int32_t gts_cluster_uses_counters(int64_t n_clusters, int32_t max_rows, int32_t max_srcs, int32_t loc_words, int32_t backward) {
   using namespace gts;
   if (n_clusters <= 0 || max_rows < 1 || max_srcs < 1 || loc_words < 0) return 0;
-  const LdsPlan p = lds_plan(max_rows, max_srcs, loc_words, backward != 0);
+  const LdsPlan p = lds_plan(max_rows, max_srcs, loc_words, backward != 0, backward == 2 ? GTS_ARG_NIBBLE : 1);
   return cluster_geometry(n_clusters, rec_layout(max_rows, max_srcs, loc_words, backward != 0).words, p.slot_bytes, p.image_off, backward != 0, false).deals ? 1 : 0;
 }
 
@@ -618,7 +643,7 @@
   using namespace gts;
   if (!rec || !x || !out || (arg_bytes != 0 && !arg)) return GTS_ERR_NULL;
   if (bad_cluster_shape(n_clusters, max_rows, max_srcs, loc_words, false, n_rows, n_feat)) return GTS_ERR_SHAPE;
-  if (arg_bytes != 0 && arg_bytes != 1) return GTS_ERR_ARGKIND;
+  if (arg_bytes != 0 && arg_bytes != 1 && arg_bytes != GTS_ARG_NIBBLE) return GTS_ERR_ARGKIND;
   if (n_clusters == 0) return GTS_OK;
   ClusterArgs a{};
   a.rec = rec, a.layout = rec_layout(max_rows, max_srcs, loc_words, false);
@@ -627,6 +652,7 @@
   a.table_bytes = static_cast<unsigned>(n_rows * kF * 4);
   a.relu_input = relu_input, a.nt = g_cluster_nt < 0 ? 1 : g_cluster_nt;
   hipStream_t st = static_cast<hipStream_t>(stream);
+  if (arg_bytes == GTS_ARG_NIBBLE) return launch_cluster<false, GTS_ARG_NIBBLE>(a, max_rows, loc_words, st);
   return arg_bytes == 0 ? launch_cluster<false, 0>(a, max_rows, loc_words, st) : launch_cluster<false, 1>(a, max_rows, loc_words, st);
 }
 
@@ -636,13 +662,15 @@
   using namespace gts;
   if (!rec || !gout || !arg || !gx) return GTS_ERR_NULL;
   if (bad_cluster_shape(n_clusters, max_rows, max_srcs, loc_words, true, n_rows, n_feat)) return GTS_ERR_SHAPE;
-  if (arg_bytes != 1) return GTS_ERR_ARGKIND;
+  if (arg_bytes != 1 && arg_bytes != GTS_ARG_NIBBLE) return GTS_ERR_ARGKIND;
   if (n_clusters == 0) return GTS_OK;
   ClusterArgs a{};
   a.rec = rec, a.layout = rec_layout(max_rows, max_srcs, loc_words, true);
   a.n_clusters = static_cast<int>(n_clusters), a.max_srcs = max_srcs;
   a.table = gout, a.winners = static_cast<const uint8_t*>(arg), a.out = gx, a.counters = counters;
-  a.table_bytes = static_cast<unsigned>(n_rows * kF * 4), a.winners_bytes = static_cast<unsigned>(n_rows * kF);
+  a.table_bytes = static_cast<unsigned>(n_rows * kF * 4);
+  a.winners_bytes = static_cast<unsigned>(arg_bytes == GTS_ARG_NIBBLE ? n_rows * kF / 2 : n_rows * kF);
   a.nt = g_cluster_nt < 0 ? 1 : g_cluster_nt;
+  if (arg_bytes == GTS_ARG_NIBBLE) return launch_cluster<true, GTS_ARG_NIBBLE>(a, max_rows, loc_words, static_cast<hipStream_t>(stream));
   return launch_cluster<true, 1>(a, max_rows, loc_words, static_cast<hipStream_t>(stream));
 }
diff --git a/gnn-tumor-seg_amd/csrc/gts_stack.hip b/gnn-tumor-seg_amd/csrc/gts_stack.hip
--- a/gnn-tumor-seg_amd/csrc/gts_stack.hip
+++ b/gnn-tumor-seg_amd/csrc/gts_stack.hip
@@ -27,6 +27,9 @@
 };
 
 inline bool packs(int64_t out_cols) { return out_cols > 128; }
+
+inline bool stack_arg_kind(int arg_bytes) { return arg_bytes == 1 || arg_bytes == 4 || arg_bytes == GTS_ARG_NIBBLE; }
+inline int64_t winner_bytes(int arg_bytes, int64_t count) { return arg_bytes == GTS_ARG_NIBBLE ? count / 2 : arg_bytes * count; }
 
 inline FwdPlan plan_forward(int64_t n, const int64_t* w, int n_layers, bool training, int arg_bytes, int flags) {
   FwdPlan p{};
@@ -36,7 +39,7 @@
     const bool last = i == n_layers - 1;
     widest = std::max(widest, w[i]);
     p.m[i] = take(4 * n * w[i]);
-    p.arg[i] = training ? take(static_cast<int64_t>(arg_bytes) * n * w[i]) : -1;
+    p.arg[i] = training ? take(winner_bytes(arg_bytes, n * w[i])) : -1;
     p.out[i] = take(4 * n * w[i + 1]);
     const bool bits = (flags & kFlagReluBits) && training && !last && gts_relu_bits_pay(n, w[i + 1]) == 1;
     p.bits[i] = bits ? take(gts_relu_bits_bytes(n, w[i + 1])) : -1;
@@ -130,7 +133,7 @@
 
 extern "C" int64_t gts_sage_pool_stack_fwd_arena(int64_t n_rows, const int64_t* widths, int32_t n_layers, int32_t training,
                                                  int32_t arg_bytes, int32_t flags, int64_t* offsets) {
-  if (bad_stack(n_rows, widths, n_layers) || (training && arg_bytes != 1 && arg_bytes != 4)) return -1;
+  if (bad_stack(n_rows, widths, n_layers) || (training && !stack_arg_kind(arg_bytes))) return -1;
   const FwdPlan p = plan_forward(n_rows, widths, n_layers, training != 0, arg_bytes, flags);
   if (offsets != nullptr) {
     for (int i = 0; i < n_layers; ++i)
@@ -148,7 +151,7 @@
                                                void* stream) {
   if (!indptr || !x || !params || !arena) return GTS_ERR_NULL;
   if (bad_stack(n_rows, widths, n_layers)) return GTS_ERR_SHAPE;
-  if (training && arg_bytes != 1 && arg_bytes != 4) return GTS_ERR_ARGKIND;
+  if (training && !stack_arg_kind(arg_bytes)) return GTS_ERR_ARGKIND;
   for (int i = 0; i < 5 * n_layers; ++i)
     if (!params[i]) return GTS_ERR_NULL;
   const bool train = training != 0;
@@ -241,7 +244,7 @@
                                                void* stream) {
   if (!t_indptr || !gout || !x || !params || !fwd_arena || !grads || !scratch) return GTS_ERR_NULL;
   if (bad_stack(n_rows, widths, n_layers)) return GTS_ERR_SHAPE;
-  if (arg_bytes != 1 && arg_bytes != 4) return GTS_ERR_ARGKIND;
+  if (!stack_arg_kind(arg_bytes)) return GTS_ERR_ARGKIND;
   for (int i = 0; i < 5 * n_layers; ++i)
     if (!params[i] || !grads[i]) return GTS_ERR_NULL;
   hipStream_t st = static_cast<hipStream_t>(stream);
@@ -261,7 +264,8 @@
   char* base = static_cast<char*>(scratch);
   auto f32 = [&](int64_t off) { return reinterpret_cast<float*>(base + off); };
   uint32_t* counters = nullptr;
-  if (sched_rec != nullptr && gts_cluster_uses_counters(sched_clusters, sched_rows, sched_srcs, sched_loc_words, 1) != 0) {
+  if (sched_rec != nullptr &&
+      gts_cluster_uses_counters(sched_clusters, sched_rows, sched_srcs, sched_loc_words, arg_bytes == GTS_ARG_NIBBLE ? 2 : 1) != 0) {
     counters = reinterpret_cast<uint32_t*>(base + plan.counters);
     if (hipMemsetAsync(counters, 0, 4 * GTS_CLUSTER_COUNTER_WORDS, static_cast<hipStream_t>(stream)) != hipSuccess) return GTS_ERR_SHAPE;
   }
@@ -330,8 +334,8 @@
       gm = buf;
     }
     float* gp = f32(plan.gp[i]);
-    if (sched_rec != nullptr && fin == 256 && arg_bytes == 1 && n_rows * 1024 < (1LL << 32)) {
-      GTS_TRY(gts_spmm_max_bwd_cluster_f32(sched_rec, sched_clusters, sched_rows, sched_srcs, sched_loc_words, gm, arg, 1, gp,
+    if (sched_rec != nullptr && fin == 256 && arg_bytes != 4 && n_rows * 1024 < (1LL << 32)) {
+      GTS_TRY(gts_spmm_max_bwd_cluster_f32(sched_rec, sched_clusters, sched_rows, sched_srcs, sched_loc_words, gm, arg, arg_bytes, gp,
                                            n_rows, fin, counters, stream));
     } else {
       GTS_TRY(gts_spmm_max_bwd_f32(t_indptr, t_indices, t_slot, gm, arg, arg_bytes, nullptr, gp, n_rows, fin, stream));
diff --git a/gnn-tumor-seg_amd/gts/nn.py b/gnn-tumor-seg_amd/gts/nn.py
--- a/gnn-tumor-seg_amd/gts/nn.py
+++ b/gnn-tumor-seg_amd/gts/nn.py
@@ -173,7 +173,8 @@
             last = i == n_layers - 1
             if p is None:
                 p = dense.linear_fwd(h, w_pool, bias=b_pool, relu=True, packed=(fragment.get(id(w_pool)), None))
-            m, arg = ops.spmm_max_fwd(g, p, want_arg=need_bwd, relu_input=True)
+            kind = ops.ARG_NIBBLE if NIBBLE_WINNERS and ops.nibble_winners_fit(g, p.shape[1]) else None
+            m, arg = ops.spmm_max_fwd(g, p, want_arg=need_bwd, relu_input=True, arg_kind=kind)
             p = None
             nxt = params[5 * (i + 1):5 * (i + 1) + 2] if not last else None
             obits = dense.relu_bits_empty(h.shape[0], w_self.shape[0], h.device) \
@@ -275,6 +276,7 @@
 
 
 STACK_IN_ONE_CALL = os.environ.get("GTS_STACK_C", "1") != "0"
+NIBBLE_WINNERS = True
 
 
 class GradSink:
@@ -348,7 +350,7 @@
         x = x.contiguous()
         n, n_layers = x.shape[0], len(params) // 5
         table, c_widths, widths = _stack_table(params, x.shape[1])
-        flags, ab = _stack_flags(), g.arg_bytes
+        flags, ab = _stack_flags(), (ops.ARG_NIBBLE if NIBBLE_WINNERS and ops.nibble_winners_fit(g, 4) else g.arg_bytes)
         d = g.dev()
         offsets = (ctypes.c_int64 * (4 * n_layers + 2))()
         total = lib.gts_sage_pool_stack_fwd_arena(n, c_widths, n_layers, 1 if need_bwd else 0, ab, flags, offsets)
diff --git a/gnn-tumor-seg_amd/gts/ops.py b/gnn-tumor-seg_amd/gts/ops.py
--- a/gnn-tumor-seg_amd/gts/ops.py
+++ b/gnn-tumor-seg_amd/gts/ops.py
@@ -3,7 +3,18 @@
 from . import _lib
 from ._lib import check, current_stream, ptr, require_device
 
-_ARG_DTYPE = {0: torch.uint8, 1: torch.uint8, 4: torch.int32}
+ARG_NIBBLE = 2
+_ARG_DTYPE = {0: torch.uint8, 1: torch.uint8, 4: torch.int32, ARG_NIBBLE: torch.uint8}
+
+
+def nibble_winners_fit(g, f):
+    return g.max_in_degree <= 14 and f % 4 == 0
+
+
+def _arg_kind(g, arg, f):
+    if arg.dtype == torch.uint8 and tuple(arg.shape) == (g.n, f // 2) and f % 4 == 0 and f > 0:
+        return ARG_NIBBLE
+    return g.arg_bytes
 
 KERNEL_TIMERS = {}
 INSTRUMENTED = False
@@ -37,7 +48,7 @@
     return buf
 
 
-def spmm_max_fwd(g, x, want_arg=True, relu_input=False):
+def spmm_max_fwd(g, x, want_arg=True, relu_input=False, arg_kind=None):
     x = x.contiguous()
     _f32(x)
     require_device(x)
@@ -46,8 +57,12 @@
         raise _lib.GtsError(f"features must be [graph nodes = {g.n}, F], got {tuple(x.shape)}")
     n, f = g.n, x.shape[1]
     out = torch.empty((n, f), dtype=torch.float32, device=x.device)
-    ab = g.arg_bytes if want_arg else 0
-    arg = torch.empty((n, f), dtype=_ARG_DTYPE[ab], device=x.device) if want_arg else None
+    ab = (g.arg_bytes if arg_kind is None else arg_kind) if want_arg else 0
+    if ab == ARG_NIBBLE and not nibble_winners_fit(g, f):
+        raise _lib.GtsError(f"4-bit winners need in-degree <= 14 and F % 4 == 0 (in-degree {g.max_in_degree}, F {f})")
+    if ab not in _ARG_DTYPE or (ab not in (0, ARG_NIBBLE) and ab != g.arg_bytes):
+        raise _lib.GtsError(f"winner kind {ab} does not belong to this graph")
+    arg = torch.empty((n, f // 2 if ab == ARG_NIBBLE else f), dtype=_ARG_DTYPE[ab], device=x.device) if want_arg else None
     lib = _lib.load()
     ds = _cluster_schedule(g, "in", n, f, ab)
     if ds is not None:
@@ -70,7 +85,7 @@
 def _cluster_schedule(g, which, n, f, arg_bytes):
     from . import schedule
 
-    if not schedule.ENABLED or f != 256 or arg_bytes not in (0, 1) or n * 1024 >= 2 ** 32 or n == 0:
+    if not schedule.ENABLED or f != 256 or arg_bytes not in (0, 1, ARG_NIBBLE) or n * 1024 >= 2 ** 32 or n == 0:
         return None
     if which == "in" and n < schedule.MIN_ROWS_FORWARD:
         return None
@@ -85,24 +100,25 @@
     if gout.dim() != 2 or gout.shape[0] != g.n:
         raise _lib.GtsError(f"gradient must be [graph nodes = {g.n}, F], got {tuple(gout.shape)}")
     n, f = g.n, gout.shape[1]
-    _expect(arg, (n, f), "arg")
+    kind = _arg_kind(g, arg, f)
+    _expect(arg, (n, f // 2 if kind == ARG_NIBBLE else f), "arg")
     _expect(relu_src, (n, f), "relu_src")
-    if arg.dtype != _ARG_DTYPE[g.arg_bytes]:
-        raise _lib.GtsError(f"arg dtype {arg.dtype} does not belong to this graph ({_ARG_DTYPE[g.arg_bytes]})")
+    if arg.dtype != _ARG_DTYPE[kind]:
+        raise _lib.GtsError(f"arg dtype {arg.dtype} does not belong to this graph ({_ARG_DTYPE[kind]})")
     gx = torch.empty((n, f), dtype=torch.float32, device=gout.device)
     lib = _lib.load()
-    ds = _cluster_schedule(g, "out", n, f, arg.element_size()) if relu_src is None else None
+    ds = _cluster_schedule(g, "out", n, f, kind) if relu_src is None else None
     if ds is not None:
         h = ds.host
 
         def launch():
             return lib.gts_spmm_max_bwd_cluster_f32(ptr(ds.packed), h.n_clusters, h.limits[0], h.limits[1], h.loc_words,
-                                                    ptr(gout), ptr(arg), 1, ptr(gx), n, f, ptr(cluster_counters(gout.device)),
+                                                    ptr(gout), ptr(arg), kind, ptr(gx), n, f, ptr(cluster_counters(gout.device)),
                                                     current_stream())
     else:
         def launch():
             return lib.gts_spmm_max_bwd_f32(ptr(d.t_indptr), ptr(d.t_indices), ptr(d.t_slot), ptr(gout),
-                                            ptr(arg), arg.element_size(), ptr(relu_src), ptr(gx), n, f,
+                                            ptr(arg), kind, ptr(relu_src), ptr(gx), n, f,
                                             current_stream())
 
     check(_timed("spmm_max_bwd_f256", launch) if f == 256 else launch(), "gts_spmm_max_bwd_f32")
diff --git a/include/gts_hip.h b/include/gts_hip.h
--- a/include/gts_hip.h
+++ b/include/gts_hip.h
@@ -11,6 +11,8 @@
 #define GTS_ERR_NULL (-1)
 #define GTS_ERR_SHAPE (-2)
 #define GTS_ERR_ARGKIND (-3)
+
+#define GTS_ARG_NIBBLE 2
 
 int32_t gts_abi_version(void);
 const char* gts_error_string(int32_t code);
```

New measurement: 961.8, median of 6. No clear change (+0.5%).
